# ashawkey/nerf2mesh

Measured on AMD Instinct MI355X. Metric: train_samples_per_sec, higher is better.
Workload: dtype f32 march/composite, f16 autocast encode+MLP (reference -O recipe); 1 GPU; nerf_synthetic/lego stage-0 -O --bound 1 --dt_gamma 0, 800x800 x 100 synthetic views, num_points target 2^18/GPU (adaptive num_rays), occupancy refresh every 16 steps; diffuse_step=1000, refresh_steps_in_window=64, parallelism=single GPU, occupancy_refresh=single GPU, mlp=fused MFMA field kernels, driver=engine.Stage0Engine (fixed launch sequence), pretrain_steps=1000, params=18367240

## Files before the change

### include/n2m_hip.h

```cpp
#ifndef N2M_HIP_H
#define N2M_HIP_H

#include <stdint.h>

#ifdef __cplusplus
extern "C" {
#endif

#define N2M_ABI_VERSION 1

enum { N2M_F32 = 0, N2M_F16 = 1 };

enum {
    N2M_OK = 0,
    N2M_EINVAL = -1,
    N2M_ENULL = -2,
    N2M_EUNSUPPORTED = -3
};

int n2m_abi_version(void);
const char* n2m_last_error(void);


int n2m_near_far_from_aabb(const float* rays_o, const float* rays_d, const float* aabb, uint32_t N,
// ... 104 lines not shown

uint64_t n2m_grid_binned_workspace_bytes(uint32_t B, uint32_t D, uint32_t C, uint32_t max_level,
                                         const int32_t* host_offsets, int dtype, int tv);
int n2m_grid_encode_backward_binned(const void* grad, const float* inputs, const int32_t* host_offsets,
                                    void* grad_embeddings, uint32_t B, uint32_t D, uint32_t C, uint32_t L,
                                    uint32_t max_level, float S, uint32_t H, uint32_t gridtype, int align_corners,
                                    uint32_t interp, int dtype, const float* tv_embeddings, float tv_weight,
                                    float tv_weight_outer, float tv_inner01, const float* tv_scale,
                                    float* found_inf, void* workspace, uint64_t workspace_bytes, void* stream);
int n2m_grad_total_variation_binned(const float* inputs, const float* embeddings, float* grad,
                                    const int32_t* host_offsets, float weight, float weight_outer, float inner01,
                                    const float* weight_scale, uint32_t B, uint32_t D, uint32_t C, uint32_t L, float S,
                                    uint32_t H, uint32_t gridtype, int align_corners, void* workspace,
                                    uint64_t workspace_bytes, void* stream);

int n2m_grid_encode_forward_pair(const float* inputs, const float* embeddings1, const void* embeddings2,
                                 const int32_t* offsets, float* outputs1, void* outputs2, uint32_t B, uint32_t L,
                                 uint32_t max_level, float S, uint32_t H, uint32_t gridtype, int align_corners,
                                 uint32_t interp, float in_scale, float in_offset, void* stream);

int n2m_grid_encode_forward_packed(const float* inputs, const void* packed, const int32_t* offsets, float* outputs1,
                                   void* outputs2, uint32_t B, uint32_t L, uint32_t max_level, float S, uint32_t H,
                                   uint32_t gridtype, int align_corners, uint32_t interp, float in_scale, float in_offset,
                                   void* stream);
int n2m_grid_encode_forward_packed_tv(const float* inputs, const void* packed, const int32_t* offsets, float* outputs1,
                                      void* outputs2, uint32_t B, uint32_t L, uint32_t max_level, float S, uint32_t H,
                                      uint32_t gridtype, int align_corners, uint32_t interp, float in_scale, float in_offset,
                                      float* tv_corners, void* stream);
int n2m_grid_encode_forward_packed_tvterms(const float* inputs, const void* packed, const int32_t* offsets, float* outputs1,
                                           void* outputs2, uint32_t B, uint32_t L, uint32_t max_level, float S, uint32_t H,
                                           uint32_t gridtype, int align_corners, uint32_t interp, float in_scale, float in_offset,
                                           float tv_weight, float tv_weight_outer, float tv_inner01, const float* tv_scale,
                                           float* tv_out, void* stream);
int n2m_grid_backward_tv_corners(const float* tv_corners);

int n2m_grid_encode_forward_packed_levels(const float* inputs, const void* packed, const int32_t* offsets, float* outputs1,
                                          void* outputs2, uint32_t B, uint32_t L, uint32_t max_level, float S, uint32_t H,
                                          uint32_t gridtype, int align_corners, uint32_t interp, float in_scale, float in_offset,
                                          uint32_t level_begin, uint32_t n_levels, void* stream);

uint64_t n2m_grid_binned_pair_workspace_bytes(uint32_t B, uint32_t max_level, const int32_t* host_offsets);
int n2m_grid_encode_backward_binned_pair(const float* grad1, const void* grad2, const float* inputs,
                                         const int32_t* host_offsets, float* grad_embeddings1,
                                         void* grad_embeddings2, uint32_t B, uint32_t L, uint32_t max_level, float S,
                                         uint32_t H, uint32_t gridtype, int align_corners, uint32_t interp,
                                         const float* tv_embeddings, float tv_weight, float tv_weight_outer,
                                         float tv_inner01, const float* tv_scale, float* found_inf, float in_scale,
                                         float in_offset, int overwrite, void* workspace, uint64_t workspace_bytes,
                                         void* stream);
int n2m_grid_encode_backward_binned_pair_half(const float* grad1, const void* grad2, const float* inputs,
                                         const int32_t* host_offsets, float* grad_embeddings1,
                                         void* grad_embeddings2, uint32_t B, uint32_t L, uint32_t max_level, float S,
                                         uint32_t H, uint32_t gridtype, int align_corners, uint32_t interp,
                                         const float* tv_embeddings, float tv_weight, float tv_weight_outer,
                                         float tv_inner01, const float* tv_scale, float* found_inf, float in_scale,
                                         float in_offset, int overwrite, void* workspace, uint64_t workspace_bytes,
                                         void* stream, int half);

typedef struct {
    const float* p_in[2]; const float* m_in[2]; const float* v_in[2];
    float* p_out[2]; float* m_out[2]; float* v_out[2];
    void* packed;
    uint32_t first_level;
    float lr[2]; int32_t slot[2];
    double beta1, beta2; float eps;
    const float* scale; const float* bias;
// ... 238 lines not shown
    float lambda_entropy; int alpha_mode;
    float* depth; const float* gt_depth; const float* depth_weight; float lambda_depth;
    int32_t* live; uint32_t* block_live;
} N2mCompositeLoss;
int n2m_composite_loss_train(const N2mCompositeLoss* d, void* stream);

int n2m_sample_order_live_first(const int32_t* rays, const int32_t* live, const uint32_t* block_live, uint32_t N, uint32_t M,
                                uint32_t* perm, void* stream);
int n2m_grid_backward_sample_order(const uint32_t* perm);

int n2m_grid_backward_merge_levels(uint32_t levels);

#define N2M_ADAM_MAX 16
typedef struct {
    void* param[N2M_ADAM_MAX]; const void* grad[N2M_ADAM_MAX]; void* exp_avg[N2M_ADAM_MAX]; void* exp_avg_sq[N2M_ADAM_MAX];
    void* half_shadow[N2M_ADAM_MAX];
    uint32_t numel[N2M_ADAM_MAX]; float lr[N2M_ADAM_MAX]; int32_t grad_is_half[N2M_ADAM_MAX];
    int32_t shadow_mode[N2M_ADAM_MAX];
    int32_t clear_grad[N2M_ADAM_MAX];
    int32_t slot[N2M_ADAM_MAX];
    uint32_t count;
} N2mAdamDesc;
int n2m_adam_step(const N2mAdamDesc* desc, double beta1, double beta2, float eps, const float* scale,
                  const float* found_inf, const float* bias, void* stream);
#define N2M_EMA_MAX 16
typedef struct {
    void* shadow[N2M_EMA_MAX]; const void* param[N2M_EMA_MAX];
    uint32_t numel[N2M_EMA_MAX];
    uint32_t count;
} N2mEmaDesc;
int n2m_ema_update(const N2mEmaDesc* desc, float one_minus_decay, void* stream);

#define N2M_TAIL_TICKET_WORDS (64 * 32)
typedef struct {
    float* growth_tracker; float* steps;
    uint32_t participants; float growth_factor, backoff_factor, growth_interval;
    const float* loss_partial; uint32_t n_partial; uint32_t n_rays; float* loss; float* loss_sum;
    const float* extra_partial; uint32_t n_extra; float extra_scale;
    const float* extra2_partial; uint32_t n_extra2; float extra2_scale;
    uint32_t* ticket;
} N2mScalerTail;
int n2m_scaler_update_slots(float* scale, float* found_inf, float* bias, double beta1, double beta2, const N2mScalerTail* tail, void* stream);

int n2m_adam_step_scaler(const N2mAdamDesc* desc, double beta1, double beta2, float eps, float* scale, float* found_inf, float* bias,
                         const N2mScalerTail* tail, void* stream);

int n2m_sdf_offsets(const float* xyz, uint32_t M, float eps, float bound, float* pts, float* pts01, void* stream);
int n2m_sdf_alpha_forward(const float* sdf, const float* sdf6, const float* dirs, const float* ts, uint32_t M, const float* variance, float eps,
                          float cos_anneal_ratio, float* alpha, float* normal, float* eik_partial, void* stream);
int n2m_sdf_alpha_backward(const float* d_alpha, const float* sdf, const float* sdf6, const float* dirs, const float* ts, uint32_t M,
                           const float* variance, float eps, float cos_anneal_ratio, const float* seed, float eik_coef, float* d_sdf,
                           float* d_sdf6, float* var_partial, float* d_variance, float* found_inf, void* stream);


int n2m_sh_encode_forward(const float* inputs, float* outputs, uint32_t B, uint32_t D, uint32_t degree,
                          float* dy_dx, void* stream);

int n2m_sh_encode_backward(const float* grad, const float* inputs, uint32_t B, uint32_t D, uint32_t degree,
                           const float* dy_dx, float* grad_inputs, void* stream);


enum {
    N2M_K_GRID_FWD = 0, N2M_K_GRID_BWD, N2M_K_GRID_TV, N2M_K_MARCH_COUNT, N2M_K_MARCH_WRITE,
    N2M_K_COMPOSITE_FWD, N2M_K_COMPOSITE_BWD, N2M_K_NEAR_FAR, N2M_K_PACKBITS, N2M_K_MLP_FWD, N2M_K_MLP_BWD,
    N2M_K_RASTER, N2M_K_GRID_FWD_PACKED , N2M_K_ADAM,
    N2M_K_INTERP_FWD, N2M_K_INTERP_BWD, N2M_K_AA_FWD, N2M_K_AA_BWD, N2M_K_RASTER_BWD, N2M_K_COUNT
};
int n2m_prof_enable(int on);
int n2m_prof_reset(void);
int n2m_prof_read(int kernel_id, uint64_t* launches, double* total_ms, double* algo_bytes);
int n2m_prof_seen(int kernel_id, uint64_t* launches_seen);
const char* n2m_prof_name(int kernel_id);

// ... 7 lines not shown
```

### include/n2m_mlp.h

```cpp
#ifndef N2M_MLP_H
#define N2M_MLP_H

#include <stdint.h>

#ifdef __cplusplus
extern "C" {
#endif

int n2m_field_forward(const float* xyz, const float* dirs, const float* h1, const void* h2, const float* w_sigma0,
                      const float* w_sigma1, const float* w_color0, const float* w_color1, const float* w_color2,
                      const float* w_spec0, const float* w_spec1, uint32_t M, int shading, int normalize_dirs, float* sigma, float* rgb,
                      float* specular, void* stream);

int n2m_field_backward(const float* xyz, const float* dirs, const float* h1, const void* h2, const float* w_sigma0,
                       const float* w_sigma1, const float* w_color0, const float* w_color1, const float* w_color2,
                       const float* w_spec0, const float* w_spec1, uint32_t M, int shading, int normalize_dirs, const float* d_sigma,
                       const float* d_rgb, const float* d_specular, float* d_h1, void* d_h2, float* d_w_sigma0,
                       float* d_w_sigma1, float* d_w_color0, float* d_w_color1, float* d_w_color2, float* d_w_spec0,
                       float* d_w_spec1, float* found_inf, void* stream);

int n2m_field_forward_train(const float* xyz, const float* dirs, const float* h1, const void* h2, const float* w_sigma0,
                            const float* w_sigma1, const float* w_color0, const float* w_color1, const float* w_color2,
                            const float* w_spec0, const float* w_spec1, uint32_t M, int shading, int normalize_dirs, float* sigma, float* rgb,
                            float* specular, float* spec_sq_partial, void* stream);
int n2m_field_backward_train(const float* xyz, const float* dirs, const float* h1, const void* h2, const float* w_sigma0,
                             const float* w_sigma1, const float* w_color0, const float* w_color1, const float* w_color2,
                             const float* w_spec0, const float* w_spec1, uint32_t M, int shading, int normalize_dirs, const float* d_sigma,
                             const float* d_rgb, const float* d_specular, float* d_h1, void* d_h2, float* d_w_sigma0,
                             float* d_w_sigma1, float* d_w_color0, float* d_w_color1, float* d_w_color2, float* d_w_spec0,
                             float* d_w_spec1, float* found_inf, float spec_reg, const float* seed, void* stream);
uint32_t n2m_field_spec_partials(void);

typedef struct N2mDwSum {
    const float* partial;
    uint32_t n_rows, mask;
    float* dw[7];
    float* found_inf;
} N2mDwSum;
int n2m_field_backward_defer_dw(N2mDwSum* out);
int n2m_field_dw_sum(const N2mDwSum* d, void* stream);
int n2m_grid_backward_dw_rider(const N2mDwSum* d, int* carried);

uint32_t n2m_field_ind_max_dim(void);
uint64_t n2m_field_ind_workspace_bytes(uint32_t M, uint32_t R);
int n2m_field_sample_views(const int32_t* rays, const int32_t* ray_view, uint32_t N, uint32_t M, int32_t* sample_view, void* stream);
int n2m_field_forward_ind(const float* xyz, const float* dirs, const float* h1, const void* h2, const float* w_sigma0,
                          const float* w_sigma1, const float* w_color0, const float* w_color1, const float* w_color2,
                          const float* w_spec0, const float* w_spec1, const float* codes, const int32_t* sample_view, uint32_t R, uint32_t D,
                          uint32_t M, int shading, int normalize_dirs, float* sigma, float* rgb, float* specular, void* stream);
int n2m_field_forward_ind_train(const float* xyz, const float* dirs, const float* h1, const void* h2, const float* w_sigma0,
                                const float* w_sigma1, const float* w_color0, const float* w_color1, const float* w_color2,
                                const float* w_spec0, const float* w_spec1, const float* codes, const int32_t* sample_view, uint32_t R,
                                uint32_t D, uint32_t M, int shading, int normalize_dirs, float* sigma, float* rgb, float* specular,
                                float* spec_sq_partial, void* stream);
int n2m_field_backward_ind(const float* xyz, const float* dirs, const float* h1, const void* h2, const float* w_sigma0,
                           const float* w_sigma1, const float* w_color0, const float* w_color1, const float* w_color2,
                           const float* w_spec0, const float* w_spec1, const float* codes, const int32_t* sample_view, uint32_t R, uint32_t D,
                           uint32_t M, int shading, int normalize_dirs, const float* d_sigma, const float* d_rgb, const float* d_specular,
                           float* d_h1, void* d_h2, float* d_w_sigma0, float* d_w_sigma1, float* d_w_color0, float* d_w_color1,
                           float* d_w_color2, float* d_w_spec0, float* d_w_spec1, float* d_codes, void* workspace, uint64_t workspace_bytes,
                           float* found_inf, void* stream);
int n2m_field_backward_ind_train(const float* xyz, const float* dirs, const float* h1, const void* h2, const float* w_sigma0,
                                 const float* w_sigma1, const float* w_color0, const float* w_color1, const float* w_color2,
                                 const float* w_spec0, const float* w_spec1, const float* codes, const int32_t* sample_view, uint32_t R,
// ... 10 lines not shown
```

### nerf2mesh_amd/_lib.py

```python
import ctypes
import os
import threading

_HERE = os.path.dirname(os.path.abspath(__file__))
LIB_PATH = os.environ.get("N2M_HIP_LIB") or os.path.join(_HERE, "lib", "libn2m_hip.so")

_u32, _i32, _f32, _vp, _int, _u64 = ctypes.c_uint32, ctypes.c_int32, ctypes.c_float, ctypes.c_void_p, ctypes.c_int, ctypes.c_uint64

SIGNATURES = {
    "n2m_near_far_from_aabb": [_vp, _vp, _vp, _u32, _f32, _vp, _vp, _vp],
    "n2m_sph_from_ray": [_vp, _vp, _f32, _u32, _vp, _vp],
    "n2m_morton3D": [_vp, _u32, _vp, _vp],
    "n2m_morton3D_invert": [_vp, _u32, _vp, _vp],
    "n2m_packbits": [_vp, _u32, _f32, _vp, _vp],
    "n2m_packbits_dev": [_vp, _u32, _vp, _vp, _vp],
    "n2m_flatten_rays": [_vp, _u32, _u32, _vp, _vp],
    "n2m_march_rays_train": [_vp, _vp, _vp, _f32, _int, _f32, _u32, _u32, _u32, _u32, _vp, _vp, _vp, _vp, _vp, _vp, _vp, _vp, _vp],
    "n2m_march_rays_train_write": [_vp, _vp, _vp, _f32, _int, _f32, _u32, _u32, _u32, _u32, _vp, _vp, _vp, _vp, _vp, _vp, _vp, _u32, _vp],
    "n2m_march_rays_train_fused": [_vp, _vp, _vp, _f32, _int, _f32, _u32, _u32, _u32, _u32, _vp, _vp, _vp, _vp, _vp, _vp, _vp, _vp, _u32, _vp, _u64, _vp],
    "n2m_march_fused_workspace_bytes": [_u32],
    "n2m_march_fallback_count": [_vp],
    "n2m_debug_fill_times": [_int, _vp],
    "n2m_stream_copy": [_vp, _vp, _u64, _u32, _vp],
    "n2m_sample_order_live_first": [_vp, _vp, _vp, _u32, _u32, _vp, _vp],
# ... 89 lines not shown
    "n2m_uv_project": [_vp, _vp, _vp, _vp, _u32, _u32, _vp, _vp, _vp],
    "n2m_uv_sum_f64": [_vp, _u32, _vp, _vp],
    "n2m_uv_rects": [_vp, _u32, ctypes.c_double, _i32, _vp, _vp, _vp],
    "n2m_uv_shelf_pack": [_vp, _vp, _u32, _i32, _i32, _vp, _vp, _vp],
    "n2m_uv_write_vt": [_vp, _vp, _vp, _vp, _u32, ctypes.c_double, _i32, _i32, _i32, _vp, _vp],
    "n2m_uv_canvas_evict": [_vp, _vp, _u32, _i32, _i32, _vp, _vp, _vp],
    "n2m_uv_face_metrics": [_vp, _vp, _vp, _u32, _i32, _i32, _vp, _vp, _vp],
    "n2m_texture_pad_nearest": [_vp, _vp, _u32, _u32, _u32, _u32, _vp],
    "n2m_asset_shade": [_vp, _vp, _vp, _vp, _vp, _vp, _vp, _u32, _u32, _u32, _u32, _int, _int, _vp, _vp],
    "n2m_freq_encode_forward": [_vp, _u32, _u32, _u32, _u32, _vp, _vp],
    "n2m_freq_encode_backward": [_vp, _vp, _u32, _u32, _u32, _u32, _vp, _vp],
    "n2m_get_rays": [_vp, _vp, _vp, _u32, _u32, _u32, _f32, _f32, _f32, _f32, _vp, _vp, _vp, _vp, _vp],
    "n2m_batch_rays": [_vp, _vp],
    "n2m_batch_views": [_vp, _u32, _u32, _vp, _vp],
    "n2m_depth_bank_fill": [_vp, _u32, _u32, _u32, _u32, _f32, _f32, _f32, _f32, _vp, _vp],
    "n2m_capture_view": [_vp, _u32, _u32, _u32, _u32, _u32, _f32, _f32, _f32, _f32, _vp, _vp, _vp, _vp, _vp, _vp, _u32, _vp],
    "n2m_capture_box_downscale": [_vp, _u32, _u32, _u32, _u32, _vp, _vp],
    "n2m_adam_step": [_vp, ctypes.c_double, ctypes.c_double, _f32, _vp, _vp, _vp, _vp],
    "n2m_adam_step_scaler": [_vp, ctypes.c_double, ctypes.c_double, _f32, _vp, _vp, _vp, _vp, _vp],
    "n2m_ema_update": [_vp, _f32, _vp],
    "n2m_scaler_update_slots": [_vp, _vp, _vp, ctypes.c_double, ctypes.c_double, _vp, _vp],
    "n2m_sdf_offsets": [_vp, _u32, _f32, _f32, _vp, _vp, _vp],
    "n2m_sdf_alpha_forward": [_vp, _vp, _vp, _vp, _u32, _vp, _f32, _f32, _vp, _vp, _vp, _vp],
    "n2m_sdf_alpha_backward": [_vp, _vp, _vp, _vp, _vp, _u32, _vp, _f32, _f32, _vp, _f32, _vp, _vp, _vp, _vp, _vp, _vp],
    "n2m_photo_loss_forward": [_vp, _vp, _vp, _vp, _f32, _f32, _f32, _u32, _vp, _vp, _vp, _vp],
    "n2m_photo_loss_backward": [_vp, _vp, _vp, _vp, _f32, _f32, _f32, _u32, _vp, _vp, _vp, _vp],
    "n2m_sh_encode_forward": [_vp, _vp, _u32, _u32, _u32, _vp, _vp],
    "n2m_sh_encode_backward": [_vp, _vp, _u32, _u32, _u32, _vp, _vp, _vp],
    "n2m_field_forward": [_vp] * 11 + [_u32, _int, _int] + [_vp] * 4,
    "n2m_field_backward": [_vp] * 11 + [_u32, _int, _int] + [_vp] * 14,
    "n2m_field_forward_train": [_vp] * 11 + [_u32, _int, _int] + [_vp] * 5,
    "n2m_field_backward_train": [_vp] * 11 + [_u32, _int, _int] + [_vp] * 13 + [_f32, _vp, _vp],
    "n2m_field_spec_partials": [],
    "n2m_field_backward_defer_dw": [_vp],
    "n2m_field_dw_sum": [_vp, _vp],
    "n2m_grid_backward_dw_rider": [_vp, _vp],
    "n2m_field_ind_max_dim": [],
    "n2m_field_ind_workspace_bytes": [_u32, _u32],
    "n2m_field_sample_views": [_vp, _vp, _u32, _u32, _vp, _vp],
    "n2m_field_forward_ind": [_vp] * 13 + [_u32, _u32, _u32, _int, _int] + [_vp] * 4,
    "n2m_field_forward_ind_train": [_vp] * 13 + [_u32, _u32, _u32, _int, _int] + [_vp] * 5,
    "n2m_field_backward_ind": [_vp] * 13 + [_u32, _u32, _u32, _int, _int] + [_vp] * 14 + [_u64, _vp, _vp],
    "n2m_field_backward_ind_train": [_vp] * 13 + [_u32, _u32, _u32, _int, _int] + [_vp] * 14 + [_u64, _vp, _f32, _vp, _vp],
    "n2m_rasterize_forward": [_vp, _vp, _u32, _u32, _u32, _u32, _vp, _vp, _vp],
    "n2m_rasterize_backward": [_vp, _vp, _vp, _vp, _u32, _u32, _u32, _u32, _vp, _vp],
    "n2m_interpolate_forward": [_vp, _vp, _vp, _u32, _u32, _u32, _u32, _u32, _vp, _vp],
    "n2m_interpolate_backward": [_vp, _vp, _vp, _vp, _u32, _u32, _u32, _u32, _u32, _vp, _vp, _vp],
    "n2m_interpolate_backward_strided": [_vp, _vp, _vp, _vp, _u32, _u32, _u32, _u32, _u32, _u32, _vp, _vp, _vp],
    "n2m_antialias_build_topology": [_vp, _u32, _vp, _u32, _vp],
    "n2m_antialias_forward": [_vp, _vp, _vp, _vp, _vp, _u32, _u32, _u32, _u32, _u32, _u32, _vp, _vp],
    "n2m_antialias_backward": [_vp, _vp, _vp, _vp, _vp, _u32, _vp, _u32, _u32, _u32, _u32, _u32, _f32, _vp, _vp, _vp],
    "n2m_antialias_backward_seeded": [_vp, _vp, _vp, _vp, _vp, _u32, _vp, _u32, _u32, _u32, _u32, _u32, _f32, _vp, _vp, _vp],
    "n2m_to_clip": [_vp, _vp, _u32, _vp, _vp],
    "n2m_to_clip_backward": [_vp, _vp, _u32, _vp, _vp],
    "n2m_laplacian_forward": [_vp, _vp, _vp, _u32, _vp, _f32, _f32, _f32, _u32, _vp, _vp, _vp, _vp],
    "n2m_laplacian_backward": [_vp, _vp, _vp, _vp, _u32, _vp, _f32, _vp, _f32, _f32, _u32, _vp, _vp, _vp],
    "n2m_laplacian_backward_acc": [_vp, _vp, _vp, _vp, _u32, _vp, _f32, _vp, _f32, _f32, _u32, _vp, _vp, _vp],
    "n2m_mesh_losses_forward": [_vp, _vp, _u32, _vp, _u32, _f32, _f32, _vp, _vp],
    "n2m_mesh_losses_backward": [_vp, _vp, _vp, _vp, _u32, _vp, _vp, _vp, _u32, _u32, _vp, _f32, _f32, _vp, _vp],
    "n2m_mesh_losses_backward_acc": [_vp, _vp, _vp, _vp, _u32, _vp, _vp, _vp, _u32, _u32, _vp, _f32, _f32, _vp, _vp],
    "n2m_gather_rows": [_vp, _vp, _u32, _u32, _vp, _vp],
    "n2m_gather_rows_strided": [_vp, _vp, _u32, _u32, _u32, _vp, _u32, _vp],
    "n2m_scatter_rows_strided": [_vp, _vp, _u32, _u32, _u32, _vp, _u32, _vp],
    "n2m_scatter_rows": [_vp, _vp, _u32, _u32, _vp, _vp],
    "n2m_stage1_head": [_vp, _vp, _vp, _u32, _u32, _u32, _vp, _vp, _f32, _f32, _f32, _vp, _vp, _vp, _vp, _vp, _vp, _vp, _vp, _vp, _vp, _int, _vp, _vp, _vp],
    "n2m_peer_alloc": [ctypes.c_size_t, _int, ctypes.POINTER(_vp)],
    "n2m_peer_free": [_vp],
    "n2m_peer_export": [_vp, _vp],
    "n2m_peer_import": [_vp, ctypes.POINTER(_vp)],
    "n2m_peer_unmap": [_vp],
    "n2m_peer_signal": [_vp, _u32, _vp],
    "n2m_peer_wait": [_vp, _u32, _u32, _u32, _u32, _vp, _vp],
    "n2m_peer_copy": [_vp, _vp, ctypes.c_size_t, _vp],
    "n2m_peer_reduce_slices": [_vp, _vp, _u32, _u32, _vp, _vp, _vp, _vp],
    "n2m_adam_step_peer": [_vp, ctypes.c_double, ctypes.c_double, _f32, _vp, _vp, _vp, _vp, _vp],
    "n2m_grid_backward_peer_route": [_vp],
    "n2m_prof_enable": [_int],
    "n2m_prof_reset": [],
    "n2m_prof_read": [_int, ctypes.POINTER(ctypes.c_uint64), ctypes.POINTER(ctypes.c_double), ctypes.POINTER(ctypes.c_double)],
    "n2m_prof_seen": [_int, ctypes.POINTER(ctypes.c_uint64)],
}

RESTYPES = {"n2m_occupancy_update_partials": _u32, "n2m_grid_binned_workspace_bytes": _u64, "n2m_grid_binned_pair_workspace_bytes": _u64, "n2m_march_fused_workspace_bytes": _u64,
            "n2m_marching_cubes_workspace_bytes": _u64, "n2m_field_spec_partials": _u32, "n2m_field_ind_max_dim": _u32,
            "n2m_field_ind_workspace_bytes": _u64}

F32, F16 = 0, 1
ADAM_MAX = 16


class AdamDesc(ctypes.Structure):
    _fields_ = [("param", _vp * ADAM_MAX), ("grad", _vp * ADAM_MAX), ("exp_avg", _vp * ADAM_MAX), ("exp_avg_sq", _vp * ADAM_MAX),
                ("half_shadow", _vp * ADAM_MAX), ("numel", _u32 * ADAM_MAX), ("lr", _f32 * ADAM_MAX), ("grad_is_half", _i32 * ADAM_MAX),
                ("shadow_mode", _i32 * ADAM_MAX), ("clear_grad", _i32 * ADAM_MAX), ("slot", _i32 * ADAM_MAX), ("count", _u32)]


class ScalerTail(ctypes.Structure):
    _fields_ = [("growth_tracker", _vp), ("steps", _vp), ("participants", _u32), ("growth_factor", _f32), ("backoff_factor", _f32),
                ("growth_interval", _f32), ("loss_partial", _vp), ("n_partial", _u32), ("n_rays", _u32), ("loss", _vp), ("loss_sum", _vp),
                ("extra_partial", _vp), ("n_extra", _u32), ("extra_scale", _f32), ("extra2_partial", _vp), ("n_extra2", _u32),
                ("extra2_scale", _f32), ("ticket", _vp)]


class DwSum(ctypes.Structure):
    _fields_ = [("partial", _vp), ("n_rows", _u32), ("mask", _u32), ("dw", _vp * 7), ("found_inf", _vp)]


class BatchRays(ctypes.Structure):
    _fields_ = [("poses", _vp), ("uniforms", _vp), ("V", _u32), ("N", _u32), ("H", _u32), ("W", _u32), ("fx", _f32), ("fy", _f32), ("cx", _f32),
                ("cy", _f32), ("intrinsics", _vp), ("images", _vp), ("bank", _vp), ("lut", _vp), ("depth_bank", _vp), ("coords", _vp),
                ("kp_depth", _vp), ("kp_weight", _vp), ("view", _u32), ("first", _u32), ("aabb", _vp), ("min_near", _f32), ("cam_near_far", _vp),
                ("rays_o", _vp), ("rays_d", _vp), ("rgba", _vp), ("nears", _vp), ("fars", _vp), ("noises", _vp), ("bg", _vp), ("gt_depth", _vp),
                ("depth_weight", _vp), ("counter", _vp)]


class CompositeLoss(ctypes.Structure):
    _fields_ = [("sigmas", _vp), ("rgbs", _vp), ("ts", _vp), ("rays", _vp), ("M", _u32), ("N", _u32), ("T_thresh", _f32), ("gt_rgba", _vp),
                ("bg", _vp), ("bg_scalar", _f32), ("lambda_rgb", _f32), ("lambda_mask", _f32), ("grad_loss", _vp), ("weights_sum", _vp),
                ("image", _vp), ("grad_sigmas", _vp), ("grad_rgbs", _vp), ("partial", _vp), ("ticket", _vp), ("loss", _vp), ("loss_sum", _vp),
                ("lambda_entropy", _f32), ("alpha_mode", _int), ("depth", _vp), ("gt_depth", _vp), ("depth_weight", _vp), ("lambda_depth", _f32),
                ("live", _vp), ("block_live", _vp)]


EMA_MAX = 16


class EmaDesc(ctypes.Structure):
    _fields_ = [("shadow", _vp * EMA_MAX), ("param", _vp * EMA_MAX), ("numel", _u32 * EMA_MAX), ("count", _u32)]


ASSET_MAX = 8


class AssetTable(ctypes.Structure):
# ... 142 lines not shown
```

### nerf2mesh_amd/csrc/gridencoder.hip

```cpp
#include <math.h>
#include <stdlib.h>

#include <atomic>
#include <type_traits>

#include "n2m_common.hpp"
#include "../../include/n2m_peer.h"
#include "../../include/n2m_mlp.h"
#include "n2m_dw_sum.hpp"

namespace {

constexpr uint32_t kMaxLevels = 32;

struct LevelTable {
    float scale[kMaxLevels];
    uint32_t resolution[kMaxLevels];
};

__host__ LevelTable make_levels(uint32_t L, float S, uint32_t H) {
    LevelTable t;
    for (uint32_t l = 0; l < kMaxLevels; ++l) {
        const float sc = l < L ? exp2f((float)l * S) * (float)H - 1.0f : 0.0f;
        t.scale[l] = sc;
        t.resolution[l] = (uint32_t)ceilf(sc) + 1u;
    }
    return t;
}

template <uint32_t D> struct Primes;
__device__ constexpr uint32_t kPrimes[7] = {1u, 2654435761u, 805459861u, 3674653429u, 2097192037u, 1434869437u, 2165219737u};

template <uint32_t D>
struct Indexer {
    uint32_t stride[D];
    uint32_t size;
    uint32_t mask;
    bool hashed, pow2, wrap;

    __device__ __forceinline__ Indexer(uint32_t size_, uint32_t resolution, uint32_t gridtype, bool align_corners) : size(size_) {
        uint32_t s = 1;
#pragma unroll
// ... 326 lines not shown
#pragma unroll
        for (uint32_t d = 0; d < D; ++d) w *= (corner & (1u << d)) ? frac[d] : 1 - frac[d];
#pragma unroll
        for (uint32_t c = 0; c < C; ++c) accum(acc.v[c], w, g[corner].v[c]);
    }
    acc.store(out);
}

template <typename T>
__global__ void zero_levels_kernel(T* __restrict__ outputs, uint32_t B, uint32_t LC, uint32_t first, uint32_t count) {
    const uint64_t t = (uint64_t)blockIdx.x * blockDim.x + threadIdx.x;
    if (t >= (uint64_t)B * count) return;
    const uint32_t b = (uint32_t)(t / count), k = (uint32_t)(t - (uint64_t)b * count);
    outputs[(size_t)b * LC + first + k] = (T)0;
}

__device__ __forceinline__ void atomic_add_row(float* dst, const float* v, uint32_t C) {
    for (uint32_t c = 0; c < C; ++c) unsafeAtomicAdd(dst + c, v[c]);
}

struct TvParams {
    const float* table;
    float weight, weight_outer, inner01;
    const float* scale_ptr;
    uint32_t stride = 1;
    const float* corners = nullptr;
};

__device__ __forceinline__ void tv_weights(const TvParams& tv, float& w_in, float& w_out) {
    float wi = tv.weight, wo = tv.weight_outer;
    if (tv.table && tv.scale_ptr) { const float s = *tv.scale_ptr; wi *= s; wo *= s; }
    w_in = wi / 6.0f; w_out = wo / 6.0f;
}
__device__ __forceinline__ bool tv_inner(const TvParams& tv, const float (&x)[3]) {
    return fmaxf(fmaxf(fabsf(x[0] - 0.5f), fabsf(x[1] - 0.5f)), fabsf(x[2] - 0.5f)) <= tv.inner01;
}
__device__ __forceinline__ float tv_reduce6(float centre, const float (&nb)[6], const bool (&nb_ok)[6], float w) {
    float sum = 0.f, sq = 0.f;
#pragma unroll
    for (uint32_t k = 0; k < 6; ++k)
        if (nb_ok[k]) { const float dv = centre - nb[k]; sum += dv; sq += dv * dv; }
    return w * sum * __builtin_amdgcn_rsqf(sq + 1e-9f);
}

__device__ __forceinline__ float tv_term(const float* __restrict__ tab, const Indexer<3>& ix, uint32_t (&cell)[3], uint32_t here, uint32_t resolution,
                                         float w, uint32_t stride);
template <bool TVT>
__global__ void __launch_bounds__(256)
grid_forward3_packed_kernel(const float* __restrict__ inputs, const uint2* __restrict__ packed, const int32_t* __restrict__ offsets,
                            float* __restrict__ out1, _Float16* __restrict__ out2, uint32_t B, uint32_t max_level, LevelTable lv,
                            uint32_t gridtype, bool align_corners, uint32_t interp, uint32_t n_tiles, float in_scale, float in_offset,
                            uint32_t xcd_group, uint32_t level_begin, uint32_t n_levels, float4* __restrict__ tv4, TvParams tv,
                            float* __restrict__ tv_out) {
    __builtin_amdgcn_s_setprio(3);
    constexpr uint32_t D = 3;
    typedef _Float16 h2 __attribute__((ext_vector_type(2)));
    uint32_t level, tile;
    if (xcd_group == 0u) {
        level = blockIdx.x / n_tiles;
        tile = blockIdx.x - level * n_tiles;
        level += level_begin;
    } else {
        const uint32_t g = xcd_group, groups = 8u / g, per_group = n_levels / groups;
        const uint32_t xcd = blockIdx.x & 7u, k = xcd / g, j = xcd - k * g, i = blockIdx.x >> 3;
        const uint32_t tiles_per_xcd = (n_tiles + g - 1u) / g;
        const uint32_t li = i / tiles_per_xcd;
        tile = (i - li * tiles_per_xcd) * g + j;
        if (li >= per_group || tile >= n_tiles) return;
        const uint32_t pair = k + groups * (li >> 1);
        level = level_begin + ((li & 1u) ? n_levels - 1u - pair : pair);
    }
    if (level >= max_level) return;
    const uint32_t b = tile * 256 + threadIdx.x;
    if (b >= B) return;
    const uint32_t row0 = (uint32_t)offsets[level];
    const uint32_t size = (uint32_t)offsets[level + 1] - row0;
    const float scale = lv.scale[level];
    const Indexer<D> ix(size, lv.resolution[level], gridtype, align_corners);
    const uint2* __restrict__ tab = packed + (size_t)row0;
    float* o1 = out1 + (size_t)level * B + b;
    _Float16* o2 = out2 ? out2 + ((size_t)level * B + b) * 2 : nullptr;

    float x[D];
    load_point<D>(inputs, b, x);
#pragma unroll
    for (uint32_t d = 0; d < D; ++d) x[d] = x[d] * in_scale + in_offset;
// ... 40 lines not shown
            rx1[q] = ((cell[0] + 1u) ^ h) & ix.mask;
            pr[q] = *reinterpret_cast<const uint4*>(tab + (rx[q] & ~1u));
        }
        uint2 extra[4];
        if (!x_even) {
#pragma unroll
            for (uint32_t q = 0; q < 4; ++q) extra[q] = tab[rx1[q]];
        }
        if constexpr (TVT) {
            const uint32_t h00 = hy0 ^ hz0;
            if (x_even) tvm[0] = tabf[(size_t)(cell[0] > 0u ? ((cell[0] - 1u) ^ h00) & ix.mask : rx[0]) * 2u];
            tvm[1] = tabf[(size_t)(cell[1] > 0u ? (cell[0] ^ (hy0 - kPrimes[1]) ^ hz0) & ix.mask : rx[0]) * 2u];
            tvm[2] = tabf[(size_t)(cell[2] > 0u ? (cell[0] ^ hy0 ^ (hz0 - kPrimes[2])) & ix.mask : rx[0]) * 2u];
        }
#pragma unroll
        for (uint32_t q = 0; q < 4; ++q) {
            const bool odd_row = (rx[q] & 1u) != 0u;
            const uint2 lo = make_uint2(pr[q].x, pr[q].y), hi = make_uint2(pr[q].z, pr[q].w);
            g[2 * q] = odd_row ? hi : lo;
            g[2 * q + 1] = x_even ? (odd_row ? lo : hi) : extra[q];
            if constexpr (TVT) { if (q == 0u && !x_even) tvm[0] = __uint_as_float(odd_row ? lo.x : hi.x); }
        }
        if (tv4) tv4[(size_t)level * B + b] = make_float4(__uint_as_float(g[0].x), __uint_as_float(g[1].x), __uint_as_float(g[2].x), __uint_as_float(g[4].x));
    } else {
#pragma unroll
        for (uint32_t corner = 0; corner < 8; ++corner) {
            const uint32_t v[D] = {cell[0] + (corner & 1u), cell[1] + ((corner >> 1) & 1u), cell[2] + (corner >> 2)};
            g[corner] = tab[ix.row(v)];
        }
        tv_fast = false;
    }
    if constexpr (TVT) {
        float w_in, w_out;
        tv_weights(tv, w_in, w_out);
        const float w = tv_inner(tv, x) ? w_in : w_out;
        float tvv;
        if (tv_fast) {
            const float nb[6] = {__uint_as_float(g[1].x), tvm[0], __uint_as_float(g[2].x), tvm[1], __uint_as_float(g[4].x), tvm[2]};
            const bool nb_ok[6] = {cell[0] < tv_res, cell[0] > 0u, cell[1] < tv_res, cell[1] > 0u, cell[2] < tv_res, cell[2] > 0u};
            tvv = tv_reduce6(__uint_as_float(g[0].x), nb, nb_ok, w);
        } else {
            tvv = tv_term(tabf, ix, cell, ix.row(cell), tv_res, w, 2u);
        }
        tv_out[(size_t)level * B + b] = tvv;
    }
    float a1 = 0.0f;
    _Float16 a2[2] = {(_Float16)0, (_Float16)0};
#pragma unroll
    for (uint32_t corner = 0; corner < 8; ++corner) {
        float w = 1.0f;
#pragma unroll
        for (uint32_t d = 0; d < D; ++d) w *= (corner & (1u << d)) ? frac[d] : 1 - frac[d];
        const h2 c2 = __builtin_bit_cast(h2, g[corner].y);
        accum(a1, w, __uint_as_float(g[corner].x));
        accum(a2[0], w, c2.x);
        accum(a2[1], w, c2.y);
    }
    *o1 = a1;
    if (!o2) return;
    Row<_Float16, 2> r2;
    r2.v[0] = a2[0]; r2.v[1] = a2[1];
    r2.store(o2);
}

__global__ void __launch_bounds__(256)
grid_forward3_pair_kernel(const float* __restrict__ inputs, const float* __restrict__ table1, const _Float16* __restrict__ table2,
                          const int32_t* __restrict__ offsets, float* __restrict__ out1, _Float16* __restrict__ out2, uint32_t B,
// ... 3663 lines not shown
    hipStream_t s = (hipStream_t)stream;
    const BinLayout lay = make_bin_plan(B, 2, L, host_offsets, false, kPairP, 2);
    N2M_REQUIRE(lay.ok, N2M_EUNSUPPORTED, "%s: table layout not supported", fn);
    const LevelTable lv = make_levels(L, S, H);
    const TvParams tv{tv_embeddings, tv_weight, tv_weight_outer, tv_inner01, tv_scale, g_cfg_tv_stride.load()};
    N2M_PROF(N2M_K_GRID_TV, s, (double)B * (12.0 + (double)L * 7 * 4.0 + (double)L * 4.0));
    tv_terms_kernel<<<dim3(n2m_ceil_div(B, 256), L), 256, 0, s>>>(inputs, tv, B, B, lay.plan, lv, gridtype, align_corners != 0, interp, in_scale, in_offset, tv_out);
    N2M_CHECK_LAUNCH();
    return 0;
}

extern "C" int n2m_grid_encode_forward_pair(const float* inputs, const float* embeddings1, const void* embeddings2, const int32_t* offsets,
                                            float* outputs1, void* outputs2, uint32_t B, uint32_t L, uint32_t max_level, float S, uint32_t H,
                                            uint32_t gridtype, int align_corners, uint32_t interp, float in_scale, float in_offset,
                                            void* stream) {
    const char* fn = "grid_encode_forward_pair";
    if (int rc = check_dims(fn, 3, 2, L, max_level, N2M_F16)) return rc;
    N2M_REQUIRE(inputs && embeddings1 && embeddings2 && offsets && outputs1 && outputs2, N2M_ENULL, "%s: NULL tensor", fn);
    if (B == 0 || max_level == 0) return 0;
    hipStream_t s = (hipStream_t)stream;
    const LevelTable lv = make_levels(L, S, H);
    N2M_PROF(N2M_K_GRID_FWD, s, (double)B * (12.0 + (double)max_level * 8 * (4 + 4) + (double)max_level * (4 + 4)));
    const uint32_t n_tiles = n2m_ceil_div(B, 256);
    grid_forward3_pair_kernel<<<n_tiles * max_level, 256, 0, s>>>(inputs, embeddings1, (const _Float16*)embeddings2, offsets, outputs1,
                                                                 (_Float16*)outputs2, B, max_level, lv, gridtype, align_corners != 0, interp, n_tiles,
                                                                 in_scale, in_offset);
    N2M_CHECK_LAUNCH();
    return 0;
}

static int forward_packed(const float* inputs, const void* packed, const int32_t* offsets, float* outputs1, void* outputs2, uint32_t B, uint32_t L,
                          uint32_t max_level, float S, uint32_t H, uint32_t gridtype, int align_corners, uint32_t interp, float in_scale, float in_offset,
                          void* stream, uint32_t level_begin, uint32_t n_levels, float* tv_corners = nullptr, const TvParams* tvp = nullptr,
                          float* tv_out = nullptr);

extern "C" int n2m_grid_encode_forward_packed(const float* inputs, const void* packed, const int32_t* offsets, float* outputs1, void* outputs2,
                                              uint32_t B, uint32_t L, uint32_t max_level, float S, uint32_t H, uint32_t gridtype,
                                              int align_corners, uint32_t interp, float in_scale, float in_offset, void* stream) {
    return forward_packed(inputs, packed, offsets, outputs1, outputs2, B, L, max_level, S, H, gridtype, align_corners, interp, in_scale, in_offset, stream, 0u,
                          max_level);
}

extern "C" int n2m_grid_encode_forward_packed_levels(const float* inputs, const void* packed, const int32_t* offsets, float* outputs1, void* outputs2,
                                                     uint32_t B, uint32_t L, uint32_t max_level, float S, uint32_t H, uint32_t gridtype,
                                                     int align_corners, uint32_t interp, float in_scale, float in_offset, uint32_t level_begin,
                                                     uint32_t n_levels, void* stream) {
    N2M_REQUIRE(n_levels >= 1 && level_begin + n_levels <= max_level, N2M_EINVAL,
                "grid_encode_forward_packed_levels: levels [%u, %u) outside [0, %u)", level_begin, level_begin + n_levels, max_level);
    return forward_packed(inputs, packed, offsets, outputs1, outputs2, B, L, max_level, S, H, gridtype, align_corners, interp, in_scale, in_offset, stream,
                          level_begin, n_levels);
}

static int forward_packed(const float* inputs, const void* packed, const int32_t* offsets, float* outputs1, void* outputs2, uint32_t B, uint32_t L,
                          uint32_t max_level, float S, uint32_t H, uint32_t gridtype, int align_corners, uint32_t interp, float in_scale, float in_offset,
                          void* stream, uint32_t level_begin, uint32_t n_levels, float* tv_corners, const TvParams* tvp, float* tv_out) {
    const char* fn = "grid_encode_forward_packed";
    if (int rc = check_dims(fn, 3, 2, L, max_level, N2M_F16)) return rc;
    N2M_REQUIRE(inputs && packed && offsets && outputs1, N2M_ENULL, "%s: NULL tensor", fn);
    N2M_REQUIRE(((uintptr_t)packed & 15u) == 0, N2M_EINVAL, "%s: the packed table must be 16-byte aligned", fn);
    if (B == 0 || max_level == 0) return 0;
    hipStream_t s = (hipStream_t)stream;
    const LevelTable lv = make_levels(L, S, H);
    N2M_PROF_K(outputs2 ? N2M_K_GRID_FWD_PACKED : N2M_K_GRID_FWD, s,
             (outputs2 ? (double)B * (12.0 + (double)n_levels * 8 * (4 + 4) + (double)n_levels * (4 + 4))
                       : (double)B * (12.0 + (double)n_levels * 8 * 4 + (double)n_levels * 4)) + (tv_out ? (double)B * n_levels * (3 * 4.0 + 4.0) : 0.0));
    const uint32_t n_tiles = n2m_ceil_div(B, 256);
    static const uint32_t xg_env = getenv("N2M_FWD_XCD_GROUP") ? (uint32_t)atoi(getenv("N2M_FWD_XCD_GROUP")) : 4u;
    const uint32_t xg = ((n_levels == 16u || n_levels == 8u) && (xg_env == 1u || xg_env == 2u || xg_env == 4u) && n_levels % (2u * (8u / xg_env)) == 0u) ? xg_env : 0u;
    const uint32_t blocks = xg ? 8u * (n_levels / (8u / xg)) * n2m_ceil_div(n_tiles, xg) : n_tiles * n_levels;
    if (tv_out) {
        TvParams tv = *tvp;
        tv.table = reinterpret_cast<const float*>(packed);
        tv.stride = 2u;
        N2M_LAUNCH(grid_forward3_packed_kernel<true>, blocks, 256, 0, s, inputs, (const uint2*)packed, offsets, outputs1, (_Float16*)outputs2, B,
                   level_begin + n_levels, lv, gridtype, align_corners != 0, interp, n_tiles, in_scale, in_offset, xg, level_begin, n_levels,
                   (float4*)nullptr, tv, tv_out);
    } else {
        N2M_LAUNCH(grid_forward3_packed_kernel<false>, blocks, 256, 0, s, inputs, (const uint2*)packed, offsets, outputs1, (_Float16*)outputs2, B,
                   level_begin + n_levels, lv, gridtype, align_corners != 0, interp, n_tiles, in_scale, in_offset, xg, level_begin, n_levels,
                   reinterpret_cast<float4*>(tv_corners), TvParams{}, (float*)nullptr);
    }
    N2M_CHECK_LAUNCH();
    return 0;
}

extern "C" int n2m_grid_encode_forward_packed_tv(const float* inputs, const void* packed, const int32_t* offsets, float* outputs1, void* outputs2,
                                                 uint32_t B, uint32_t L, uint32_t max_level, float S, uint32_t H, uint32_t gridtype, int align_corners,
                                                 uint32_t interp, float in_scale, float in_offset, float* tv_corners, void* stream) {
    N2M_REQUIRE(tv_corners == nullptr || ((uintptr_t)tv_corners & 15u) == 0, N2M_EINVAL, "grid_encode_forward_packed_tv: tv_corners must be 16-byte aligned");
    return forward_packed(inputs, packed, offsets, outputs1, outputs2, B, L, max_level, S, H, gridtype, align_corners, interp, in_scale, in_offset, stream,
                          0u, max_level < L ? max_level : L, tv_corners);
}

extern "C" int n2m_grid_encode_forward_packed_tvterms(const float* inputs, const void* packed, const int32_t* offsets, float* outputs1, void* outputs2,
                                                      uint32_t B, uint32_t L, uint32_t max_level, float S, uint32_t H, uint32_t gridtype,
                                                      int align_corners, uint32_t interp, float in_scale, float in_offset, float tv_weight,
                                                      float tv_weight_outer, float tv_inner01, const float* tv_scale, float* tv_out, void* stream) {
    N2M_REQUIRE(tv_out != nullptr, N2M_ENULL, "grid_encode_forward_packed_tvterms: NULL tv_out");
    N2M_REQUIRE(max_level == L, N2M_EINVAL, "grid_encode_forward_packed_tvterms: TV terms need max_level == L (every level of tv_out is written)");
    const TvParams tv{nullptr, tv_weight, tv_weight_outer, tv_inner01, tv_scale, 2u};
    return forward_packed(inputs, packed, offsets, outputs1, outputs2, B, L, max_level, S, H, gridtype, align_corners, interp, in_scale, in_offset, stream,
                          0u, L, nullptr, &tv, tv_out);
}

extern "C" int n2m_debug_fill_times(int on, unsigned long long* out) {
    if (out) N2M_HIP(hipMemcpyFromSymbol(out, HIP_SYMBOL(g_fill_t), sizeof(unsigned long long) * 96));
    if (out) N2M_HIP(hipMemcpyFromSymbol(out + 96, HIP_SYMBOL(g_acc_t), sizeof(unsigned long long) * 20));
    const unsigned int v = (unsigned int)on;
    N2M_HIP(hipMemcpyToSymbol(HIP_SYMBOL(g_fill_timing_on), &v, sizeof(v)));
    g_fill_dbg_host = v;
    return 0;
}

extern "C" int n2m_grid_backward_peer_route(const N2mPeerRoute* route) {
    if (!route) { g_peer_route = N2mPeerRoute{}; return 0; }
    N2M_REQUIRE(route->world >= 1 && route->world <= N2M_PEER_MAX && route->rows_c > 0 && route->rows_f > 0 &&
                (uint64_t)route->world * route->rows_c >= route->split_row && (uint64_t)(route->world - 1u) * route->rows_c < route->split_row,
                N2M_EINVAL, "grid_backward_peer_route: 1..%d ranks, (world - 1) * rows_c < split_row <= world * rows_c", N2M_PEER_MAX);
    for (int h = 0; h < 2; ++h)
        for (uint32_t r = 0; r < route->world; ++r)
            N2M_REQUIRE(route->g1[h][r] && route->g2[h][r], N2M_ENULL, "grid_backward_peer_route: NULL staging slot (half %d, owner %u)", h, r);
    g_peer_route = *route;
    return 0;
}

extern "C" int n2m_grid_backward_config(int tv_stride, float overflow_div) {
    N2M_REQUIRE((tv_stride == 1 || tv_stride == 2) && overflow_div >= 1.0f, N2M_EINVAL, "grid_backward_config: tv_stride 1 or 2, overflow_div >= 1");
    g_cfg_tv_stride.v = (uint32_t)tv_stride;
    g_cfg_overflow_div.v = overflow_div;
    return 0;
}
```

### nerf2mesh_amd/csrc/mlp.hip

```cpp
#include <map>
#include <mutex>

#include "n2m_common.hpp"
#include "../../include/n2m_mlp.h"
#include "n2m_dw_sum.hpp"

namespace {

typedef _Float16 h4 __attribute__((ext_vector_type(4)));
typedef float f16x __attribute__((ext_vector_type(16)));

#define MFMA(a, b, c) __builtin_amdgcn_mfma_f32_32x32x8f16((a), (b), (c), 0, 0, 0)
typedef _Float16 h8 __attribute__((ext_vector_type(8)));
#define MFMA16(a, b, c) __builtin_amdgcn_mfma_f32_32x32x16_f16((a), (b), (c), 0, 0, 0)

constexpr int P_S0 = 28, P_S1 = 36, P_C0 = 44, P_C1 = 68, P_C2 = 68, P_P0 = 12, P_P1 = 36;
constexpr int P_S1T = 12, P_S0T = 36, P_C2T = 12, P_C1T = 68, P_C0T = 68, P_P1T = 12, P_P0T = 36;
constexpr int O_S0 = 0;
constexpr int O_S1 = O_S0 + 32 * P_S0;
constexpr int O_C0 = O_S1 + 32 * P_S1;
constexpr int O_C1 = O_C0 + 64 * P_C0;
constexpr int O_C2 = O_C1 + 64 * P_C1;
constexpr int O_P0 = O_C2 + 32 * P_C2;
constexpr int O_P1 = O_P0 + 32 * P_P0;
constexpr int FWD_HALVES = O_P1 + 32 * P_P1;
constexpr int O_S1T = FWD_HALVES;
constexpr int O_S0T = O_S1T + 32 * P_S1T;
constexpr int O_C2T = O_S0T + 32 * P_S0T;
constexpr int O_C1T = O_C2T + 64 * P_C2T;
constexpr int O_C0T = O_C1T + 64 * P_C1T;
constexpr int O_P1T = O_C0T + 64 * P_C0T;
constexpr int O_P0T = O_P1T + 32 * P_P1T;
constexpr int ALL_W_HALVES = O_P0T + 32 * P_P0T;
constexpr int TILE_PITCH = 68;
constexpr int TILE_HALVES = 32 * TILE_PITCH;
constexpr int BWD_HALVES = ALL_W_HALVES + 4 * 2 * TILE_HALVES;
constexpr int BWD_PC_TILES_HALVES = ALL_W_HALVES + 4 * 4 * TILE_HALVES;
constexpr int BWD_PC_HALVES = BWD_PC_TILES_HALVES > 65536 ? BWD_PC_TILES_HALVES : 65536;
// ... 312 lines not shown
    for (int i = 0; i < 8; ++i) { asm volatile("" : "+v"(r.h1v[i])); asm volatile("" : "+v"(r.h2v[i])); }
#pragma unroll
    for (int i = 0; i < 3; ++i) { asm volatile("" : "+v"(r.xyz[i])); asm volatile("" : "+v"(r.dir[i])); asm volatile("" : "+v"(r.drgb[i])); asm volatile("" : "+v"(r.dspec[i])); }
    asm volatile("" : "+v"(r.dsig));
}
__device__ __forceinline__ void density_frags(const RawTile& r, h4 (&b)[3]) {
#pragma unroll
    for (int kb = 0; kb < 2; ++kb)
#pragma unroll
        for (int i = 0; i < 4; ++i) b[kb][i] = (_Float16)r.h1v[4 * kb + i];
    b[2] = zero4();
    b[2][0] = (_Float16)r.xyz[0]; b[2][1] = (_Float16)r.xyz[1]; b[2][2] = (_Float16)r.xyz[2];
}
__device__ __forceinline__ void color_frags(const RawTile& r, h4 (&b)[5]) {
#pragma unroll
    for (int kb = 0; kb < 4; ++kb) {
        const u2v_t v = {r.h2v[2 * kb], r.h2v[2 * kb + 1]};
        b[kb] = __builtin_bit_cast(h4, v);
    }
    b[4] = zero4();
    b[4][0] = (_Float16)r.xyz[0]; b[4][1] = (_Float16)r.xyz[1]; b[4][2] = (_Float16)r.xyz[2];
}
template <typename P>
__device__ __forceinline__ void dir_frag(const FieldArgs& a, const RawTile& r, P& bp) {
    float d0 = r.dir[0], d1 = r.dir[1], d2 = r.dir[2];
    if (a.normalize_dirs) {
        const float nn = sqrtf(fmaxf((d0 * d0 + d1 * d1) + d2 * d2, 1e-20f));
        d0 /= nn; d1 /= nn; d2 /= nn;
    }
    bp[0] = (_Float16)d0; bp[1] = (_Float16)d1; bp[2] = (_Float16)d2;
}

template <bool DO_DENSITY, bool DO_COLOR, bool IND = false>
__global__ void __launch_bounds__(256) field_forward_kernel(typename ArgsOf<IND>::type a) {
    __builtin_amdgcn_s_setprio(3);
    extern __shared__ __attribute__((aligned(16))) _Float16 lds[];
    stage_images<256, false, DO_DENSITY, DO_COLOR, IND>(lds, a);
    if constexpr (IND) stage_color0_ind<false>(lds + O_C0X_FWD, nullptr, a.w[2], a.ind.D);

    const int lane = threadIdx.x & 63, n = lane & 31, g = lane >> 5;
    const uint32_t wave = blockIdx.x * 4 + (threadIdx.x >> 6), n_waves = gridDim.x * 4;
    const uint32_t n_tiles = (a.M + 31) / 32;
    RawTile nxt;
    float spec_sq = 0.f;
    fetch_tile<DO_DENSITY, DO_COLOR, false>(a, wave, n, g, nxt);
    for (uint32_t tile = wave; tile < n_tiles; tile += n_waves) {
        const uint32_t s = tile * 32 + n;
        const bool valid = s < a.M;
        settle_tile(nxt);
        const RawTile cur = nxt;
        fetch_tile<DO_DENSITY, DO_COLOR, false>(a, tile + n_waves, n, g, nxt);
        if (DO_DENSITY) {
            h4 b0[3];
            density_frags(cur, b0);
            f16x d = zero16();
            d = mm_k<3>(lds + O_S0, P_S0, 0, b0, d, lane);
            const h4 b1[4] = {relu_pack<0>(d), relu_pack<1>(d), relu_pack<2>(d), relu_pack<3>(d)};
            f16x o = zero16();
            o = mm_k<4>(lds + O_S1, P_S1, 0, b1, o, lane);
            if (valid && g == 0) a.sigma[s] = a.raw_density ? (float)(_Float16)o[0] : expf((float)(_Float16)o[0]);
        }
        if (DO_COLOR) {
            h4 b0[5];
            color_frags(cur, b0);
            f16x d1[2] = {zero16(), zero16()};
            h4 bc[2];
            if constexpr (IND) code_frags(a.ind, s, valid, g, bc);
#pragma unroll
            for (int mb = 0; mb < 2; ++mb) {
                if constexpr (IND) {
                    d1[mb] = mm_k<5>(lds + O_C0X_FWD, P_C0X, mb, b0, d1[mb], lane);
                    d1[mb] = MFMA16(cat8(ld_a(lds + O_C0X_FWD, P_C0X, mb, 5, lane), ld_a(lds + O_C0X_FWD, P_C0X, mb, 6, lane)), cat8(bc[0], bc[1]), d1[mb]);
                } else
                d1[mb] = mm_k<5>(lds + O_C0, P_C0, mb, b0, d1[mb], lane);
// ... 14 lines not shown
                h4 bp = zero4();
                if (g == 0) {
                    if (valid) dir_frag(a, cur, bp);
                    bp[3] = (_Float16)q3;
                } else { bp[0] = (_Float16)q0; bp[1] = (_Float16)q1; }
                f16x p1 = MFMA(ld_a(lds + O_P0, P_P0, 0, 0, lane), bp, zero16());
                const h4 bq[4] = {relu_pack<0>(p1), relu_pack<1>(p1), relu_pack<2>(p1), relu_pack<3>(p1)};
                f16x p2 = zero16();
                p2 = mm_k<4>(lds + O_P1, P_P1, 0, bq, p2, lane);
                const float s0 = sigmoid_h(p2[0]), s1 = sigmoid_h(p2[1]), s2 = sigmoid_h(p2[2]);
                if (valid && g == 0 && a.specular) {
                    a.specular[(size_t)s * 3] = s0; a.specular[(size_t)s * 3 + 1] = s1; a.specular[(size_t)s * 3 + 2] = s2;
                }
                if (valid && g == 0) spec_sq += (s0 * s0 + s1 * s1) + s2 * s2;
                if (a.shading == 2) { cr = s0; cg = s1; cb = s2; }
                else {
                    cr = fminf(fmaxf((float)(_Float16)(s0 + q0), 0.f), 1.f);
                    cg = fminf(fmaxf((float)(_Float16)(s1 + q1), 0.f), 1.f);
                    cb = fminf(fmaxf((float)(_Float16)(s2 + q2), 0.f), 1.f);
                }
            }
            if (valid && g == 0 && a.rgb) {
                a.rgb[(size_t)s * 3] = cr; a.rgb[(size_t)s * 3 + 1] = cg; a.rgb[(size_t)s * 3 + 2] = cb;
            }
        }
    }
    if (DO_COLOR && a.spec_sq_partial) {
        __shared__ float spec_wave[4];
        const float w = n2m_wave_sum(spec_sq);
        if (lane == 0) spec_wave[threadIdx.x >> 6] = w;
        __syncthreads();
        if (threadIdx.x == 0) a.spec_sq_partial[blockIdx.x] = ((spec_wave[0] + spec_wave[1]) + spec_wave[2]) + spec_wave[3];
        if (blockIdx.x == 0)
            for (int i = (int)gridDim.x + (int)threadIdx.x; i < kSpecPartials; i += 256) a.spec_sq_partial[i] = 0.f;
    }
}

__device__ __forceinline__ void tile_put(_Float16* tile, int kb, const h4& f, int lane) {
    *reinterpret_cast<h4*>(tile + (lane & 31) * TILE_PITCH + 8 * kb + 4 * (lane >> 5)) = f;
}
__device__ __forceinline__ h4 tile_get(const _Float16* tile, int kq, int fb, int lane) {
    const _Float16* p = tile + (8 * kq + 4 * (lane >> 5)) * TILE_PITCH + 32 * fb + (lane & 31);
    h4 r;
    r[0] = p[0]; r[1] = p[TILE_PITCH]; r[2] = p[2 * TILE_PITCH]; r[3] = p[3 * TILE_PITCH];
    return r;
}
typedef short s4v_t __attribute__((__vector_size__(8)));
__device__ __forceinline__ h4 tile_get_tr(const _Float16* tile, int kq, int fb, int lane) {
    const _Float16* p = tile + (8 * kq + 4 * (lane >> 5) + ((lane & 15) >> 2)) * TILE_PITCH + 32 * fb + 16 * ((lane >> 4) & 1) + 4 * (lane & 3);
    return __builtin_bit_cast(h4, __builtin_amdgcn_ds_read_tr16_b64_v4i16((__attribute__((address_space(3))) s4v_t*)p));
}
template <int MB, int NB, bool TR = false>
__device__ __forceinline__ void dw_tile(f16x (&acc)[MB][NB], const _Float16* tY, const _Float16* tX, int lane) {
    if constexpr (TR) {
        h4 ay[4][MB], bx[4][NB];
#pragma unroll
        for (int kq = 0; kq < 4; ++kq) {
#pragma unroll
            for (int mb = 0; mb < MB; ++mb) ay[kq][mb] = tile_get_tr(tY, kq, mb, lane);
#pragma unroll
            for (int nb = 0; nb < NB; ++nb) bx[kq][nb] = tile_get_tr(tX, kq, nb, lane);
        }
#pragma unroll
        for (int kq = 0; kq < 4; kq += 2)
#pragma unroll
            for (int mb = 0; mb < MB; ++mb)
#pragma unroll
                for (int nb = 0; nb < NB; ++nb)
// ... 633 lines not shown
}

int check_field(const char* fn, const float* xyz, const float* h1, const float* const* w, bool density, int shading) {
    N2M_REQUIRE(shading >= 0 && shading <= 2, N2M_EINVAL, "%s: shading must be 0 (diffuse), 1 (full) or 2 (specular)", fn);
    N2M_REQUIRE(xyz, N2M_ENULL, "%s: xyz is NULL", fn);
    if (density) N2M_REQUIRE(h1 && w[0] && w[1], N2M_ENULL, "%s: density branch needs h1 and sigma_net weights", fn);
    return 0;
}

float* dw_scratch(hipStream_t s, bool ind = false) {
    static std::mutex mu;
    static std::map<std::pair<int, hipStream_t>, float*> plain, wide;
    auto& bufs = ind ? wide : plain;
    std::lock_guard<std::mutex> lk(mu);
    int dev = 0;
    if (hipGetDevice(&dev) != hipSuccess) return nullptr;
    const auto key = std::make_pair(dev, s);
    auto it = bufs.find(key);
    if (it != bufs.end()) return it->second;
    float* p = nullptr;
    if (hipMalloc((void**)&p, (size_t)256 * (ind ? kDwTotalInd : kDwTotal) * sizeof(float)) != hipSuccess) return nullptr;
    bufs[key] = p;
    return p;
}

uint32_t persistent_grid(uint32_t M) {
    const uint32_t tiles = (M + 31) / 32;
    const uint32_t need = (tiles + 3) / 4;
    return need < 256u ? (need ? need : 1u) : 256u;
}

}

static int field_forward_impl(const float* xyz, const float* dirs, const float* h1, const void* h2, const float* w_sigma0,
                                 const float* w_sigma1, const float* w_color0, const float* w_color1, const float* w_color2,
                                 const float* w_spec0, const float* w_spec1, uint32_t M, int shading, int normalize_dirs, float* sigma, float* rgb,
                                 float* specular, float* spec_sq_partial, void* stream, const IndArgs* ind = nullptr) {
    const float* w[7] = {w_sigma0, w_sigma1, w_color0, w_color1, w_color2, w_spec0, w_spec1};
    const bool density = sigma != nullptr;
    if (int rc = check_field("field_forward", xyz, h1, w, density, shading)) return rc;
    const bool color = rgb != nullptr;
    N2M_REQUIRE(density || color, N2M_ENULL, "field_forward: both sigma and rgb are NULL");
    if (color) {
        N2M_REQUIRE(h2 && w[2] && w[3] && w[4], N2M_ENULL, "field_forward: colour branch needs h2 and color_net weights");
        if (shading != 0) N2M_REQUIRE(dirs && w[5] && w[6], N2M_ENULL, "field_forward: shading != 0 needs dirs and specular_net weights");
    }
    if (M == 0) return 0;
    FieldArgs a{};
    a.xyz = xyz; a.dirs = dirs; a.h1 = h1; a.h2 = (const _Float16*)h2; a.normalize_dirs = normalize_dirs & 1; a.raw_density = (normalize_dirs >> 1) & 1;
    for (int i = 0; i < 7; ++i) a.w[i] = w[i];
    a.M = M; a.shading = shading; a.sigma = sigma; a.rgb = rgb; a.specular = specular;
    a.spec_sq_partial = (color && shading != 0) ? spec_sq_partial : nullptr;
    hipStream_t s = (hipStream_t)stream;
    N2M_PROF_K(N2M_K_MLP_FWD, s, (double)M * (12 + 64 + 4 + (color ? 64 + 12 + 12 + 12 : 0)));
    const size_t smem = (size_t)FWD_HALVES * 2;
    if (ind && color) {
        FieldArgsInd ai{};
        static_cast<FieldArgs&>(ai) = a;
        ai.ind = *ind;
        const size_t smem_ind = (size_t)(FWD_HALVES + C0X_HALVES) * 2;
        if (density) N2M_LAUNCH((field_forward_kernel<true, true, true>), persistent_grid(M) * 2, 256, smem_ind, s, ai);
        else N2M_LAUNCH((field_forward_kernel<false, true, true>), persistent_grid(M) * 2, 256, smem_ind, s, ai);
        N2M_CHECK_LAUNCH();
        return 0;
    }
    if (color && density) N2M_LAUNCH((field_forward_kernel<true, true>), persistent_grid(M) * 2, 256, smem, s, a);
    else if (color) N2M_LAUNCH((field_forward_kernel<false, true>), persistent_grid(M) * 2, 256, smem, s, a);
    else N2M_LAUNCH((field_forward_kernel<true, false>), persistent_grid(M) * 2, 256, smem, s, a);
    N2M_CHECK_LAUNCH();
    return 0;
}

extern "C" int n2m_field_forward(const float* xyz, const float* dirs, const float* h1, const void* h2, const float* w_sigma0,
                                 const float* w_sigma1, const float* w_color0, const float* w_color1, const float* w_color2,
                                 const float* w_spec0, const float* w_spec1, uint32_t M, int shading, int normalize_dirs, float* sigma, float* rgb,
                                 float* specular, void* stream) {
    return field_forward_impl(xyz, dirs, h1, h2, w_sigma0, w_sigma1, w_color0, w_color1, w_color2, w_spec0, w_spec1, M, shading, normalize_dirs,
                              sigma, rgb, specular, nullptr, stream);
}
extern "C" int n2m_field_forward_train(const float* xyz, const float* dirs, const float* h1, const void* h2, const float* w_sigma0,
                                       const float* w_sigma1, const float* w_color0, const float* w_color1, const float* w_color2,
                                       const float* w_spec0, const float* w_spec1, uint32_t M, int shading, int normalize_dirs, float* sigma,
                                       float* rgb, float* specular, float* spec_sq_partial, void* stream) {
    return field_forward_impl(xyz, dirs, h1, h2, w_sigma0, w_sigma1, w_color0, w_color1, w_color2, w_spec0, w_spec1, M, shading, normalize_dirs,
                              sigma, rgb, specular, spec_sq_partial, stream);
}
extern "C" uint32_t n2m_field_spec_partials(void) { return (uint32_t)kSpecPartials; }

static thread_local N2mDwSum* g_defer_dw = nullptr;
extern "C" int n2m_field_backward_defer_dw(N2mDwSum* out) {
    g_defer_dw = out;
    if (out) *out = N2mDwSum{};
    return 0;
}
static int check_dw_sum(const char* fn, const N2mDwSum* d) {
    N2M_REQUIRE(d != nullptr && d->partial != nullptr, N2M_ENULL, "%s: NULL description / partial rows", fn);
    N2M_REQUIRE(d->n_rows >= 1, N2M_EINVAL, "%s: no partial rows", fn);
    N2M_REQUIRE((d->mask & ~0x7Fu) == 0, N2M_EINVAL, "%s: mask names seven tensors", fn);
    for (int i = 0; i < 7; ++i)
        N2M_REQUIRE(!((d->mask >> i) & 1u) || d->dw[i] != nullptr, N2M_ENULL, "%s: tensor %d is in the mask and NULL", fn, i);
    return 0;
}
extern "C" int n2m_field_dw_sum(const N2mDwSum* d, void* stream) {
    if (int rc = check_dw_sum("field_dw_sum", d)) return rc;
    DwOut o;
    for (int i = 0; i < 7; ++i) o.dw[i] = d->dw[i];
    N2M_LAUNCH(dw_finalize_kernel, kDwSumBlocks, 1024, 0, (hipStream_t)stream, d->partial, d->n_rows, o, d->mask, d->found_inf);
    N2M_CHECK_LAUNCH();
    return 0;
}

static int field_backward_impl(const float* xyz, const float* dirs, const float* h1, const void* h2, const float* w_sigma0,
                                  const float* w_sigma1, const float* w_color0, const float* w_color1, const float* w_color2,
                                  const float* w_spec0, const float* w_spec1, uint32_t M, int shading, int normalize_dirs, const float* d_sigma,
                                  const float* d_rgb, const float* d_specular, float* d_h1, void* d_h2, float* d_w_sigma0,
                                  float* d_w_sigma1, float* d_w_color0, float* d_w_color1, float* d_w_color2, float* d_w_spec0,
                                  float* d_w_spec1, float* found_inf, float spec_reg, const float* seed, void* stream,
                                  const IndArgs* ind = nullptr, float* d_codes = nullptr, long long* code_acc = nullptr) {
// ... 181 lines not shown
```

### nerf2mesh_amd/csrc/step_helpers.hip

```cpp
#include <string.h>

#include "n2m_common.hpp"
#include "../../include/n2m_peer.h"

namespace {

struct RayTerm {
    float e[3];
    float m;
    float bg[3];
};

__device__ __forceinline__ RayTerm ray_term(const float* __restrict__ image, const float* __restrict__ wsum,
                                            const float* __restrict__ gt, const float* __restrict__ bg, float bg_scalar, uint32_t r) {
    RayTerm t;
    const float4 g = *reinterpret_cast<const float4*>(gt + (size_t)r * 4);
    const float a = g.w, ws = wsum[r];
    const float gc[3] = {g.x, g.y, g.z};
#pragma unroll
    for (int c = 0; c < 3; ++c) {
        t.bg[c] = bg ? bg[(size_t)r * 3 + c] : bg_scalar;
        const float target = gc[c] * a + t.bg[c] * (1.0f - a);
        const float pred = image[(size_t)r * 3 + c] + (1.0f - ws) * t.bg[c];
        t.e[c] = pred - target;
    }
    t.m = ws - a;
    return t;
}

__global__ void __launch_bounds__(256)
photo_loss_forward_kernel(const float* __restrict__ image, const float* __restrict__ wsum, const float* __restrict__ gt,
                          const float* __restrict__ bg, float bg_scalar, float lambda_rgb, float lambda_mask, uint32_t N,
                          float* __restrict__ partial, uint32_t* __restrict__ ticket, float* __restrict__ loss) {
    __shared__ float wave_sum[4];
    __shared__ bool last;
    const uint32_t r = blockIdx.x * 256 + threadIdx.x, lane = threadIdx.x & 63u, wid = threadIdx.x >> 6;
// ... 801 lines not shown
                               const float* gt_rgba, const float* bg, float bg_scalar, float lambda_rgb, float lambda_mask, float* image,
                               float* depth, float* weights_sum, float* trig_id, float* loss_px, float* d_alpha, float* d_rgb, float* partial,
                               float* tri_err, float* tri_cnt, int packed_rgba, const float* seed, float* d_copy, void* stream) {
    N2M_REQUIRE(aa_alpha && aa_rgb && rast && gt_rgba && image && depth && weights_sum && trig_id && loss_px && partial, N2M_ENULL,
                "stage1_head: NULL tensor");
    N2M_REQUIRE((d_alpha == nullptr) == (d_rgb == nullptr), N2M_ENULL, "stage1_head: d_alpha and d_rgb come together");
    N2M_REQUIRE((tri_err == nullptr) == (tri_cnt == nullptr), N2M_ENULL, "stage1_head: tri_err and tri_cnt come together");
    N2M_REQUIRE(ssaa == 1 || ssaa == 2, N2M_EUNSUPPORTED, "stage1_head: ssaa 1 or 2 (the reduction is the exact 2 x 2 mean of torch's bilinear minification)");
    N2M_REQUIRE(h0 > 0 && w0 > 0 && (uint64_t)h0 * w0 < (1ull << 31), N2M_EINVAL, "stage1_head: bad image size");
    N2M_REQUIRE(!packed_rgba || !d_rgb || (d_alpha == d_rgb + 3 && ((uintptr_t)d_rgb & 15u) == 0), N2M_EINVAL,
                "stage1_head: packed gradients are ONE 16-byte aligned [h, w, 4] image (d_alpha = d_rgb + 3)");
    N2M_REQUIRE(!d_copy || (packed_rgba && d_rgb && ((uintptr_t)d_copy & 15u) == 0), N2M_EINVAL, "stage1_head: d_copy goes with the packed gradient image");
    hipStream_t s = (hipStream_t)stream;
    const uint32_t N = h0 * w0;
    if (ssaa == 1)
        stage1_head_kernel<1><<<n2m_ceil_div(N, 256), 256, 0, s>>>(aa_alpha, aa_rgb, rast, h0, w0, gt_rgba, bg, bg_scalar, lambda_rgb, lambda_mask,
                                                                  image, depth, weights_sum, trig_id, loss_px, d_alpha, d_rgb, partial, tri_err, tri_cnt, packed_rgba ? 4u : 1u,
                                                                  packed_rgba ? 4u : 3u, seed, d_copy);
    else
        stage1_head_kernel<2><<<n2m_ceil_div(N, 256), 256, 0, s>>>(aa_alpha, aa_rgb, rast, h0, w0, gt_rgba, bg, bg_scalar, lambda_rgb, lambda_mask,
                                                                  image, depth, weights_sum, trig_id, loss_px, d_alpha, d_rgb, partial, tri_err, tri_cnt, packed_rgba ? 4u : 1u,
                                                                  packed_rgba ? 4u : 3u, seed, d_copy);
    N2M_CHECK_LAUNCH();
    return 0;
}

template <bool PEER>
__global__ void __launch_bounds__(256)
adam_kernel(AdamTensors t, float beta1, float beta2, float omb1, float omb2, float eps, const float* scale, const float* found_inf,
            const float* bias, AdamPeerK pe) {
    adam_body<PEER>(t, beta1, beta2, omb1, omb2, eps, scale, found_inf, bias, pe);
}

struct ScalerTailK {
    float* scale; float* growth_tracker; float* found_inf; float* steps; float* bias;
    uint32_t participants; double beta1, beta2; float growth_factor, backoff_factor, growth_interval;
    const float* loss_partial; uint32_t n_partial; float inv_rays; float* loss; float* loss_sum;
    const float* extra_partial; uint32_t n_extra; float extra_scale;
    const float* extra2_partial; uint32_t n_extra2; float extra2_scale;
    uint32_t* ticket;
};

template <bool ONE_WAVE>
__device__ __forceinline__ void scaler_update_slots_body(const ScalerTailK& k) {
    const uint32_t s = ONE_WAVE ? (threadIdx.x & 63u) : threadIdx.x;
    float tot_part = 0.0f, tot_extra = 0.0f, tot_extra2 = 0.0f;
    bool ok;
    if constexpr (ONE_WAVE) {
        auto sum256 = [&](const float* __restrict__ part, uint32_t n) {
            float acc[4] = {0.0f, 0.0f, 0.0f, 0.0f};
            for (uint32_t base = 0; base < n; base += 2048u) {
                float x[8][4];
#pragma unroll
                for (uint32_t k = 0; k < 8u; ++k)
#pragma unroll
                    for (uint32_t w = 0; w < 4u; ++w) {
                        const uint32_t i = base + 256u * k + 64u * w + s;
                        x[k][w] = i < n ? part[i] : 0.0f;
                    }
#pragma unroll
                for (uint32_t k = 0; k < 8u; ++k)
#pragma unroll
                    for (uint32_t w = 0; w < 4u; ++w)
                        if (base + 256u * k + 64u * w + s < n) acc[w] += x[k][w];
            }
            float tot = 0.0f;
#pragma unroll
            for (uint32_t w = 0; w < 4u; ++w) tot += n2m_wave_sum(acc[w]);
            return tot;
        };
        if (k.extra2_partial) tot_extra2 = sum256(k.extra2_partial, k.n_extra2);
        if (k.extra_partial) tot_extra = sum256(k.extra_partial, k.n_extra);
        if (k.loss_partial) tot_part = sum256(k.loss_partial, k.n_partial);
        ok = *k.found_inf == 0.0f;
    } else {
        __shared__ float wave_part[16], wave_extra[16], wave_extra2[16];
        if (k.extra2_partial) {
            float acc = 0.0f;
            for (uint32_t i = s; i < k.n_extra2; i += blockDim.x) acc += k.extra2_partial[i];
            acc = n2m_wave_sum(acc);
            if ((s & 63u) == 0u) wave_extra2[s >> 6] = acc;
        }
        if (k.extra_partial) {
            float acc = 0.0f;
            for (uint32_t i = s; i < k.n_extra; i += blockDim.x) acc += k.extra_partial[i];
            acc = n2m_wave_sum(acc);
            if ((s & 63u) == 0u) wave_extra[s >> 6] = acc;
        }
        if (k.loss_partial) {
            float acc = 0.0f;
            for (uint32_t i = s; i < k.n_partial; i += blockDim.x) acc += k.loss_partial[i];
            acc = n2m_wave_sum(acc);
            if ((s & 63u) == 0u) wave_part[s >> 6] = acc;
        }
        ok = *k.found_inf == 0.0f;
        __syncthreads();
        if (s == 0) {
            for (uint32_t w = 0; w < (blockDim.x + 63u) / 64u; ++w) {
                if (k.loss_partial) tot_part += wave_part[w];
                if (k.extra_partial) tot_extra += wave_extra[w];
                if (k.extra2_partial) tot_extra2 += wave_extra2[w];
            }
        }
    }
    if (k.loss_partial && s == 0) {
        float v = tot_part * k.inv_rays;
        if (k.extra_partial) v += tot_extra * k.extra_scale;
        if (k.extra2_partial) v += tot_extra2 * k.extra2_scale;
        if (k.loss) *k.loss = v;
        if (k.loss_sum) *k.loss_sum += v;
    }
    if (s == 0) {
        if (!ok) {
            if (k.scale) *k.scale *= k.backoff_factor;
            if (k.growth_tracker) *k.growth_tracker = 0.0f;
        } else if (k.growth_tracker) {
            const float g = *k.growth_tracker + 1.0f;
            if (g >= k.growth_interval) {
                const float ns = *k.scale * k.growth_factor;
                if (k.scale && ns <= 3.0e38f) *k.scale = ns;
                *k.growth_tracker = 0.0f;
            } else {
                *k.growth_tracker = g;
            }
        }
        *k.found_inf = 0.0f;
    }
    if (s <= N2M_ADAM_MAX) {
        if (ok && (s == 0 || ((k.participants >> (s - 1u)) & 1u))) k.steps[s] += 1.0f;
        const double t = (double)k.steps[s] + 1.0;
        k.bias[2u * s] = (float)(1.0 - pow(k.beta1, t));
        k.bias[2u * s + 1u] = (float)sqrt(1.0 - pow(k.beta2, t));
    }
}


constexpr uint32_t kTailSlots = 64;
struct AdamTailArgs {
    AdamTensors t; float beta1, beta2, omb1, omb2, eps; const float* scale; const float* found_inf; const float* bias; ScalerTailK tail;
};

__global__ void __launch_bounds__(256) __attribute__((amdgpu_num_sgpr(48)))
adam_kernel_with_scaler(AdamTensors t, float beta1, float beta2, float omb1, float omb2, float eps, const float* scale, const float* found_inf,
                        const float* bias, ScalerTailK tail) {
    adam_body<false>(t, beta1, beta2, omb1, omb2, eps, scale, found_inf, bias, AdamPeerK{});
    if (blockIdx.x != gridDim.x - 1u || threadIdx.x >= 64u) {
        if ((threadIdx.x & 63u) == 0u)
            (void)__hip_atomic_fetch_add(tail.ticket + 32u * (blockIdx.x & (kTailSlots - 1u)), 1u, __ATOMIC_RELAXED, __HIP_MEMORY_SCOPE_AGENT);
        return;
    }
    uint32_t off = (uint32_t)offsetof(AdamTailArgs, tail);
    asm volatile("" : "+s"(off));
    const ScalerTailK* tp = reinterpret_cast<const ScalerTailK*>((const char*)__builtin_amdgcn_kernarg_segment_ptr() + off);
    {
        const uint32_t expected = 4u * gridDim.x - 1u;
        uint32_t* mine = tp->ticket + 32u * threadIdx.x;
        for (;;) {
            uint32_t v = 0u;
#pragma unroll
            for (uint32_t k = 0; k < kTailSlots / 64u; ++k) v += __hip_atomic_load(mine + 32u * 64u * k, __ATOMIC_RELAXED, __HIP_MEMORY_SCOPE_AGENT);
            if (n2m_wave_sum_u32(v) >= expected) break;
            __builtin_amdgcn_s_sleep(8);
        }
#pragma unroll
        for (uint32_t k = 0; k < kTailSlots / 64u; ++k) __hip_atomic_store(mine + 32u * 64u * k, 0u, __ATOMIC_RELAXED, __HIP_MEMORY_SCOPE_AGENT);
    }
    const ScalerTailK k = *tp;
    scaler_update_slots_body<true>(k);
}

static ScalerTailK scaler_tail_k(float* scale, float* found_inf, float* bias, double beta1, double beta2, const N2mScalerTail* t) {
    const bool lp = t->loss_partial != nullptr;
    const float* e1 = lp ? t->extra_partial : nullptr;
    const float* e2 = lp ? t->extra2_partial : nullptr;
    return ScalerTailK{scale, t->growth_tracker, found_inf, t->steps, bias, t->participants, beta1, beta2, t->growth_factor, t->backoff_factor,
                       t->growth_interval, t->loss_partial, lp ? t->n_partial : 0u, lp ? 1.0f / (float)t->n_rays : 0.0f, lp ? t->loss : nullptr,
                       lp ? t->loss_sum : nullptr, e1, e1 ? t->n_extra : 0u, t->extra_scale, e2, e2 ? t->n_extra2 : 0u, t->extra2_scale, t->ticket};
}

static int adam_step_impl(const N2mAdamDesc* d, double beta1, double beta2, float eps, const float* scale, const float* found_inf,
                          const float* bias, const N2mAdamPeer* peer, void* stream, const N2mScalerTail* tail = nullptr) {
    N2M_REQUIRE(d != nullptr && bias != nullptr, N2M_ENULL, "adam_step: NULL descriptor / bias");
    N2M_REQUIRE(d->count >= 1 && d->count <= N2M_ADAM_MAX, N2M_EINVAL, "adam_step: 1..%d tensors per call (got %u)", N2M_ADAM_MAX, d->count);
    AdamTensors t;
    memset(&t, 0, sizeof(t));
    uint32_t blocks = 0;
    for (uint32_t k = 0; k < d->count; ++k) {
        N2M_REQUIRE(d->param[k] && d->grad[k] && d->exp_avg[k] && d->exp_avg_sq[k], N2M_ENULL, "adam_step: NULL tensor %u", k);
        N2M_REQUIRE((((uintptr_t)d->param[k] | (uintptr_t)d->grad[k] | (uintptr_t)d->exp_avg[k] | (uintptr_t)d->exp_avg_sq[k]) & 3u) == 0,
                    N2M_EINVAL, "adam_step: tensor %u is not 4-byte aligned (param/grad/exp_avg/exp_avg_sq)", k);
        t.p[k] = (uint64_t)d->param[k]; t.g[k] = (uint64_t)d->grad[k]; t.m[k] = (uint64_t)d->exp_avg[k]; t.v[k] = (uint64_t)d->exp_avg_sq[k];
        t.shadow[k] = (uint64_t)d->half_shadow[k];
        t.n[k] = d->numel[k];
        t.lr[k] = d->lr[k];
        t.first_block[k] = blocks;
        blocks += n2m_ceil_div(d->numel[k], 1024);
        if (d->grad_is_half[k]) t.g_half_mask |= 1u << k;
        if (d->clear_grad[k] && !d->grad_is_half[k]) t.clear_mask |= 1u << k;
        t.shadow_mode[k] = (uint8_t)(d->half_shadow[k] ? (d->shadow_mode[k] ? d->shadow_mode[k] : 1) : 0);
        N2M_REQUIRE(d->slot[k] >= 0 && d->slot[k] <= N2M_ADAM_MAX, N2M_EINVAL, "adam_step: slot of tensor %u out of range", k);
        t.slot[k] = (uint8_t)d->slot[k];
        N2M_REQUIRE(t.shadow_mode[k] <= 3 && !(t.shadow_mode[k] == 3 && (d->numel[k] & 1u)), N2M_EINVAL, "adam_step: bad shadow mode for tensor %u", k);
    }
    for (uint32_t k = 0; k < d->count; ++k) t.partner[k] = -1;
    for (uint32_t k = 0; k < d->count; ++k) {
        if (t.shadow_mode[k] != 3) continue;
        for (uint32_t j = 0; j < d->count; ++j)
            if (t.shadow_mode[j] == 2 && d->half_shadow[j] == d->half_shadow[k] && d->numel[k] == 2 * d->numel[j] && ((uintptr_t)d->half_shadow[k] & 15u) == 0) {
                N2M_REQUIRE(!((t.clear_mask >> j) & 1u), N2M_EUNSUPPORTED,
                            "adam_step: tensor %u shares a packed table with tensor %u and cannot use clear_grad", j, k);
                t.partner[k] = (int8_t)j;
// ... 62 lines not shown
                                                                        found_inf, bias, pe);
        else
            N2M_LAUNCH((adam_kernel<false>), blocks, 256, 0, (hipStream_t)stream, t, (float)beta1, (float)beta2, (float)(1.0 - beta1), (float)(1.0 - beta2), eps, scale,
                                                                         found_inf, bias, pe);
    }
    N2M_CHECK_LAUNCH();
    return 0;
}

extern "C" int n2m_adam_step(const N2mAdamDesc* d, double beta1, double beta2, float eps, const float* scale, const float* found_inf,
                             const float* bias, void* stream) {
    return adam_step_impl(d, beta1, beta2, eps, scale, found_inf, bias, nullptr, stream);
}

extern "C" int n2m_adam_step_scaler(const N2mAdamDesc* d, double beta1, double beta2, float eps, float* scale, float* found_inf, float* bias,
                                    const N2mScalerTail* tail, void* stream) {
    N2M_REQUIRE(tail != nullptr, N2M_ENULL, "adam_step_scaler: NULL tail (use n2m_adam_step + n2m_scaler_update_slots)");
    return adam_step_impl(d, beta1, beta2, eps, scale, found_inf, bias, nullptr, stream, tail);
}

extern "C" int n2m_adam_step_peer(const N2mAdamDesc* d, double beta1, double beta2, float eps, const float* scale, const float* found_inf,
                                  const float* bias, const N2mAdamPeer* peer, void* stream) {
    N2M_REQUIRE(peer != nullptr, N2M_ENULL, "adam_step_peer: NULL peer description (use n2m_adam_step)");
    return adam_step_impl(d, beta1, beta2, eps, scale, found_inf, bias, peer, stream);
}

__global__ void scaler_update_slots_kernel(const ScalerTailK k) {
    __builtin_amdgcn_s_setprio(3);
    scaler_update_slots_body<false>(k);
}

extern "C" int n2m_scaler_update_slots(float* scale, float* found_inf, float* bias, double beta1, double beta2, const N2mScalerTail* tail,
                                       void* stream) {
    N2M_REQUIRE(tail != nullptr, N2M_ENULL, "scaler_update_slots: NULL tail");
    N2M_REQUIRE(found_inf != nullptr && tail->steps != nullptr && bias != nullptr, N2M_ENULL, "scaler_update_slots: NULL found_inf / steps / bias");
    N2M_REQUIRE(tail->loss_partial == nullptr || tail->n_rays > 0, N2M_EINVAL, "scaler_update_slots: the loss partials need the ray count");
    scaler_update_slots_kernel<<<1, tail->loss_partial ? 256 : 64, 0, (hipStream_t)stream>>>(scaler_tail_k(scale, found_inf, bias, beta1, beta2, tail));
    N2M_CHECK_LAUNCH();
    return 0;
}

struct EmaTensors {
    uint64_t shadow[N2M_EMA_MAX], param[N2M_EMA_MAX];
    uint32_t n[N2M_EMA_MAX], first_block[N2M_EMA_MAX + 1];
    uint32_t count;
};

__global__ void __launch_bounds__(256) ema_update_kernel(EmaTensors t, float one_minus_decay) {
    uint32_t k = 0;
    while (k + 1 < t.count && blockIdx.x >= t.first_block[k + 1]) ++k;
    const uint32_t i0 = ((blockIdx.x - t.first_block[k]) * 256u + threadIdx.x) * 4u;
    const uint32_t n = t.n[k];
    if (i0 >= n) return;
    float* __restrict__ S = reinterpret_cast<float*>(t.shadow[k]);
    const float* __restrict__ P = reinterpret_cast<const float*>(t.param[k]);
    typedef float f4v __attribute__((ext_vector_type(4)));
    if (i0 + 4u <= n && (((t.shadow[k] | t.param[k]) & 15u) == 0)) {
        f4v s = __builtin_nontemporal_load(reinterpret_cast<const f4v*>(S + i0));
        const f4v p = __builtin_nontemporal_load(reinterpret_cast<const f4v*>(P + i0));
        s.x = s.x - (s.x - p.x) * one_minus_decay; s.y = s.y - (s.y - p.y) * one_minus_decay;
        s.z = s.z - (s.z - p.z) * one_minus_decay; s.w = s.w - (s.w - p.w) * one_minus_decay;
        __builtin_nontemporal_store(s, reinterpret_cast<f4v*>(S + i0));
    } else {
        for (uint32_t e = 0; e < 4u && i0 + e < n; ++e) S[i0 + e] = S[i0 + e] - (S[i0 + e] - P[i0 + e]) * one_minus_decay;
    }
}

extern "C" int n2m_ema_update(const N2mEmaDesc* d, float one_minus_decay, void* stream) {
    N2M_REQUIRE(d != nullptr, N2M_ENULL, "ema_update: NULL descriptor");
// ... 22 lines not shown
```

### nerf2mesh_amd/engine.py

```python
import ctypes
import os
import time

import numpy as np
import torch

from . import _lib as L
from . import raymarching, synthetic
from .fused import SHADING, _affine
from .gridencoder import _host_offsets, same_geometry
from .optim import FusedAdamAMP

_p = L.ptr


def _shard_refresh_default():
    from .parallel import shard_refresh_default
    return shard_refresh_default()


def lr_lambda(it, iters):
    return 0.01 + 0.99 * (it / 500) if it <= 500 else 0.1 ** ((it - 500) / (iters - 500))


def peer_chunk_rows(split, world, pad=0):
    if split % 4 != 0 or pad % 4 != 0:
        return None
    cs = (split + 4 * world - 1) // (4 * world) * 4 + pad
    return cs if (world - 1) * cs < split else None


class _RayBufs:

    def __init__(self, cap, dev):
        self.cap = cap
        f = lambda *s: torch.empty(*s, dtype=torch.float32, device=dev)
        self.o, self.d, self.rgba = f(cap, 3), f(cap, 3), f(cap, 4)
        self.nears, self.fars, self.noises, self.bg_buf = f(cap), f(cap), f(cap), f(cap, 3)
        self.gtd, self.dw = f(cap), f(cap)
        self.depth_view = None
        self.u = self.bg = None
        self.rays = torch.empty(cap, 2, dtype=torch.int32, device=dev)
        self.views = None
        self.counter = torch.zeros(1, dtype=torch.int32, device=dev)
        self.ws = torch.empty(int(L.lib().n2m_march_fused_workspace_bytes(cap)), dtype=torch.uint8, device=dev)
        self.one_pass = False
        self.host_count = torch.empty(1, dtype=torch.int32, pin_memory=True)
        self.count_ready = torch.cuda.Event()
        self.written = torch.cuda.Event()
        self.spec = False
        self.index = 0
        self.M = None
        self.loss = torch.empty(1, dtype=torch.float32, device=dev)
        self.samples = None
        self.cap_m = 0
        self.N = 0
        self.args = None
        self.refreshed = False


class Stage0Engine:
    def __init__(self, model, opt, poses, device, rank=0, world_size=1, seed=0, ema_decay=0.95, capture=None):
        self.model, self.opt, self.device = model.to(device), opt, torch.device(device)
        dev = self.device
        self.capture = capture
        if capture is not None:
            capture.check_device(dev)
            poses = capture.poses
        assert dev.type == "cuda", "the step executor drives HIP kernels: no CPU path"
        if bool(opt.sdf) and world_size > 1:
            raise ValueError("Stage0Engine runs the SDF recipe on one rank; use trainer.Stage0Trainer for multi-rank SDF training")
        self.ind_dim = int(getattr(opt, "ind_dim", 0))
        if self.ind_dim > 0 and capture is not None and len(capture) > int(opt.ind_num):
            raise ValueError(f"the capture has {len(capture)} views but ind_num is {int(opt.ind_num)}: every view needs a code row")
        if not self.supported(model, opt, capture=capture, world_size=world_size):
            raise ValueError("Stage0Engine covers the fused recipes (fused_mlp, fp16, individual codes only on a capture -- density mode, "
                             "one rank, ind_dim <= 16 --, power-of-two bound, shared encoder geometry); use trainer.Stage0Trainer for "
                             "other configurations")
        L.lib()
        self.poses = poses.to(dev).float().contiguous()
        self.rank, self.world = rank, world_size
        self.global_step = 0
        self.num_rays = opt.num_rays
        self.gen = torch.Generator(device=dev)
        self.gen.manual_seed(seed + rank)
        self.optimizer = FusedAdamAMP(model.get_params(opt.lr), eps=1e-15, amp=True)
        self.ema = None
        self.epoch_len = max(1, int(poses.shape[0]))
        if ema_decay is not None:
            from .ema import ExponentialMovingAverage
            self.ema = ExponentialMovingAverage(model.parameters(), decay=ema_decay)
# ... 94 lines not shown
                f32 = lambda *sh: torch.empty(*sh, dtype=torch.float32, device=dev)
                f16 = lambda *sh: torch.empty(*sh, dtype=torch.float16, device=dev)
                self.g1s = {"c": f32(self._Cs, 1), "f": f32(self._Fs, 1)}
                self.g2s = {"c": f16(self._Cs, 2), "f": f16(self._Fs, 2)}
                self._inplace_gather = dist.get_backend() == "nccl"
                self.chunked_gather = os.environ.get("N2M_CHUNKED_GATHER", "1") != "0"
        self._bwd_cfg = (2 if self.shard else 1, float(world_size))
        self.peer = None
        if self.shard and os.environ.get("N2M_PEER_STORE", "0") == "1":
            if opt.sdf:
                raise ValueError("N2M_PEER_STORE covers the NeRF recipes (the SDF head's folded backward is not routed)")
            from .parallel import PeerExchange
            self.peer = PeerExchange(rank, world_size, self.rows, self._split, self._Cs, self._Fs, dev, small_n=self.dw.numel() + 1)
            self._peer_small = torch.empty(self.dw.numel() + 1, dtype=torch.float32, device=dev)
            pk = model.packed_tables()
            self.peer.packed.copy_(pk)
            model._packed = self.peer.packed
            model._packed_buffer = self.peer.packed
            self._peer_route = self.peer.route()
            self._peer_fused = (os.environ.get("N2M_PEER_FUSED", "1") != "0" and self._Cs % 4 == 0 and self._Fs % 4 == 0 and self._split % 2 == 0)
            self._adam_peer = None
        if self.shard:
            self.optimizer.shard_sync = lambda: self.sync_parameters(moments=True)
        self.sdf_fold = os.environ.get("N2M_SDF_FOLD", "1") != "0"
        self.sdf_tv_all = os.environ.get("N2M_SDF_TV_ALL", "1") != "0"
        self.fuse_adam = None
        if world_size == 1 and not opt.sdf and self.Lv == 16 and os.environ.get("N2M_FUSE_ADAM", "0") == "1":
            fl, fr = ctypes.c_uint32(0), ctypes.c_uint32(0)
            self._fuse_cap = 1 << 19
            L.call("n2m_grid_pair_fuse_plan", self._fuse_cap, self.Lv, self.ho.ctypes.data, ctypes.byref(fl), ctypes.byref(fr))
            if fl.value < self.Lv:
                self.fuse_adam = {"first_level": int(fl.value), "first_row": int(fr.value), "alt": None, "desc": {}}
                self._bwd_cfg = (2, 1.0)

    @staticmethod
    def supported(model, opt, capture=None, world_size=1):
        e1, e2 = model.encoder, model.encoder_color
        sdf = bool(opt.sdf)
        from .fused import ind_max_dim
        ind = int(getattr(opt, "ind_dim", 0))
        ind_ok = ind == 0 or (capture is not None and not sdf and world_size == 1 and ind <= ind_max_dim())
        return (bool(getattr(opt, "fused_mlp", False)) and bool(opt.fp16) and ind_ok
                and _affine(float(model.bound)) is not None and same_geometry(e1, e2) and e1.embeddings.shape[1] == 1
                and e2.embeddings.shape[1] == 2 and (sdf or not getattr(opt, "progressive_level", False))
                and opt.patch_size == 1 and (sdf or model.max_level >= e1.num_levels) and not (sdf and opt.lambda_entropy > 0)
                and not (sdf and (getattr(opt, "enable_sparse_depth", False) or getattr(opt, "enable_dense_depth", False))))

    @property
    def loss_acc(self):
        return self._loss_sum

    def _lambda_mask(self):
        if self.capture is not None and not self.capture.has_alpha:
            return 0.0
        return float(max(self.opt.lambda_mask, 0.0))

    def mark_untrained(self):
        if self.opt.mark_untrained and self.capture is not None:
            self.model.mark_untrained_grid(self.poses, self.capture.intrinsics, cam_near_far=self.cam_near_far)
        elif self.opt.mark_untrained:
            f = synthetic.LEGO_FOCAL
            self.model.mark_untrained_grid(self.poses, (f, f, synthetic.LEGO_HW / 2, synthetic.LEGO_HW / 2), cam_near_far=self.cam_near_far)

    def _ray_bufs(self, N):
        self._cur = (self._cur + 1) % len(self._bufs)
        b = self._bufs[self._cur]
        if b is None or b.cap < N:
            b = self._bufs[self._cur] = _RayBufs(max(int(N * 1.5), self._min_rays), self.device)
        return b

    def _sample_bufs(self, b, cap_m):
        if b.samples is None or b.cap_m < cap_m:
            b.cap_m = int(cap_m)
            b.samples = torch.empty(b.cap_m * 8, dtype=torch.float32, device=self.device)
        c = b.cap_m
        s = b.samples
        return s[:3 * c], s[3 * c:6 * c], s[6 * c:]

    def _work(self, M, N):
        cm, cn = self._work_cap
        if M > cm or N > cn:
            cm, cn = max(cm, int(M * 1.25) + 1024), max(cn, int(N * 1.5) + 1024, self._depth_rays)
            dev = self.device
# ... 352 lines not shown

    @torch.no_grad()
    def sync_parameters(self, density_only=False, moments=False):
        if not self.shard:
            return
        self._wait_gather()
        if self.peer is not None:
            self.peer.check()
        done = getattr(self, "_synced", (-1, False, False))
        level = (not density_only, moments)
        if done[0] == self.global_step and (done[1] or density_only) and (done[2] or not moments):
            return
        self._synced = (self.global_step, level[0] or (done[0] == self.global_step and done[1]), level[1] or (done[0] == self.global_step and done[2]))
        import torch.distributed as dist
        e1p, e2p = self.model.encoder.embeddings, self.model.encoder_color.embeddings
        tables = [(e1p.data, 1)] if density_only else [(e1p.data, 1), (e2p.data, 2)]
        if moments:
            for p, C in ((e1p, 1), (e2p, 2)):
                st = self.optimizer.state[p]
                tables += [(st["exp_avg"], C), (st["exp_avg_sq"], C)]
        for t, C in tables:
            flat = t.view(-1)
            for h, (row0, n) in self._shard_ranges().items():
                lo = 0 if h == "c" else self._split
                if h == "c" and getattr(self, "_uneven", False):
                    for r in range(self.world):
                        r0, rn = self._shard_ranges_of(r)["c"]
                        if rn > 0:
                            dist.broadcast(flat[r0 * C:(r0 + rn) * C], src=r)
                    continue
                dist.all_gather_into_tensor(flat[lo * C:(lo + self.world * n) * C], flat[row0 * C:(row0 + n) * C].clone())

    def _scaler_tail(self, participants, loss_out):
        o = self.optimizer
        gf, bf, gi = o.growth
        tail = L.ScalerTail(growth_tracker=_p(o.growth_tracker), steps=_p(o.steps), participants=participants, growth_factor=gf, backoff_factor=bf,
                            growth_interval=gi, ticket=_p(self._tail_ticket))
        if loss_out is not None:
            n_rays, buf, extra = loss_out[:3]
            ex_buf, ex_scale = extra if extra is not None else (None, 0.0)
            e2_buf, e2_n, e2_scale = loss_out[3] if len(loss_out) > 3 and loss_out[3] is not None else (None, 0, 0.0)
            tail.loss_partial, tail.n_partial, tail.n_rays, tail.loss, tail.loss_sum = _p(self._w["partial"]), (n_rays + 15) // 16, n_rays, _p(buf), _p(self._loss_sum)
            tail.extra_partial, tail.n_extra, tail.extra_scale = _p(ex_buf), self._n_spec, float(ex_scale)
            tail.extra2_partial, tail.n_extra2, tail.extra2_scale = _p(e2_buf), int(e2_n), float(e2_scale)
        return tail

    def _optimizer_step(self, full, lr_factor, loss_out=None, fused=None):
        o = self.optimizer
        self._wait_gather()
        desc, participants, groups = self._adam_desc(full, dense_only=fused is not None)
        for k, gi in enumerate(groups):
            desc.lr[k] = float(o.param_groups[gi]["initial_lr"]) * lr_factor
        b1, b2 = o.param_groups[0]["betas"]
        s = L.stream()
        peer_fused = self.peer is not None and self._peer_fused
        scaler_done = False
        if self.lookup_overlap and fused is None and not self.shard and self.Lv == 16:
            d_f, d_c = self._adam_desc_halves(full, lr_factor)
            for d in (d_f, d_c):
                L.call("n2m_adam_step", ctypes.addressof(d), float(b1), float(b2), float(o.param_groups[0]["eps"]), _p(o.scale), _p(o.found_inf),
                       _p(o.bias), s)
                if d is d_f:
                    self._fine_ready = torch.cuda.Event()
                    self._fine_ready.record()
        elif peer_fused:
            if self._adam_peer is None:
                self._adam_peer = self.peer.adam_peer([("s1", "c"), ("s2", "c"), ("s1", "f"), ("s2", "f")] + [None] * (desc.count - 4))
            L.call("n2m_adam_step_peer", ctypes.addressof(desc), float(b1), float(b2), float(o.param_groups[0]["eps"]), _p(o.scale), _p(o.found_inf),
                   _p(o.bias), ctypes.addressof(self._adam_peer), s)
        elif (self.adam_tail and loss_out is not None and fused is None and self.peer is None and not self.shard):
            tail = self._scaler_tail(participants, loss_out)
            L.call("n2m_adam_step_scaler", ctypes.addressof(desc), float(b1), float(b2), float(o.param_groups[0]["eps"]), _p(o.scale), _p(o.found_inf),
                   _p(o.bias), ctypes.addressof(tail), s)
            scaler_done = True
        else:
            L.call("n2m_adam_step", ctypes.addressof(desc), float(b1), float(b2), float(o.param_groups[0]["eps"]), _p(o.scale), _p(o.found_inf),
                   _p(o.bias), s)
        self.model.encoder_color._half_version = -1
        if fused is not None:
            L.call("n2m_adam_fuse_restore", ctypes.addressof(fused), self.ho.ctypes.data, self.Lv, _p(o.found_inf), s)
            self._fuse_swap()
        if self.peer is not None:
            for h, (row0, n) in self._shard_ranges().items():
                if peer_fused:
                    self.peer.signal_rows(h)
                else:
                    self.peer.push_rows(h, row0, n)
            self._gathers = self.peer.rows_tokens()
            if not self.chunked_gather:
                self._wait_gather()
        elif self.shard:
            self._gather_packed()
        if not scaler_done:
            tail = self._scaler_tail(participants, loss_out)
            L.call("n2m_scaler_update_slots", _p(o.scale), _p(o.found_inf), _p(o.bias), float(b1), float(b2), ctypes.addressof(tail), s)
        nxt = lr_lambda(self.global_step, self.opt.iters)
        for group in o.param_groups:
            group["lr"] = float(group["initial_lr"]) * nxt

    @torch.no_grad()
    def train_step(self):
        opt, model, dev = self.opt, self.model, self.device
        if not model.training:
            model.train()
        for g in self.optimizer.param_groups:
            g.setdefault("initial_lr", g["lr"])
        if not self._queue:
            self._fill_pipeline()
        b = self._queue.pop(0)
        self.global_step += 1
        assert b.index == self.global_step
        N = b.N
        random_bg = b.bg is not None
        bg = b.bg
        shading = SHADING["diffuse" if (self.global_step < opt.diffuse_step or opt.diffuse_only) else "full"]
        M = self._finish(b)
        self.last_num_points = M
        self.samples_seen += M
        self.rays_seen += N

        if opt.sdf:
            opt.cos_anneal_ratio = min(1, self.global_step / (0.5 * opt.iters))
            opt.normal_anneal_epsilon = 1e-1 * (1 - min(0.999, self.global_step / (0.5 * opt.iters)))
            if opt.progressive_level:
                model.max_level = 4 + int(12 * min(1, self.global_step / (0.5 * opt.iters)))
        w = self._work(max(M, 1), N)
        s = L.stream()
        c = b.cap_m
        xyzs = dirs = ts = None
        if M > 0:
            xyzs, dirs, ts = b.samples[:3 * c], b.samples[3 * c:6 * c], b.samples[6 * c:]
        o = self.optimizer
        pk = model.packed_tables()
        if self.lookup_overlap and getattr(self, "_packed", None) is not None and pk.data_ptr() != self._packed.data_ptr():
            self._fine_ready = None
        sw = self.mlp_params
        e1 = model.encoder
        seed = o.scale if self.world == 1 else o.scale / self.world
        if opt.sdf:
            return self._step_sdf(b, M, N, w, xyzs, dirs, ts, shading, seed, pk)
        fwd_terms = False
        if M > 0:
            fwd = (_p(xyzs), _p(pk), _p(e1.offsets), _p(w["h1"]), _p(w["h2"]), M, self.Lv, self.Lv, self.S, self.H0, e1.gridtype_id,
                   int(bool(e1.align_corners)), e1.interp_id, float(self.aff[0]), float(self.aff[1]))
            if self.shard and getattr(self, "_gathers", None) and self.Lv == 16:
                self._wait_gather(("c",))
                L.call("n2m_grid_encode_forward_packed_levels", *fwd, 0, 8, s)
                self._wait_gather(("f",))
                L.call("n2m_grid_encode_forward_packed_levels", *fwd, 8, 8, s)
            elif self.lookup_overlap and self._fine_ready is not None and self.Lv == 16:
                self.s_lookup.wait_event(self._fine_ready)
                with torch.cuda.stream(self.s_lookup):
                    L.call("n2m_grid_encode_forward_packed_levels", *fwd, 8, 8, L.stream())
                    done = torch.cuda.Event()
                    done.record()
                L.call("n2m_grid_encode_forward_packed_levels", *fwd, 0, 8, s)
                torch.cuda.current_stream(dev).wait_event(done)
            elif self.tv_corners and self.Lv == 16 and self.fuse_adam is None:
                L.call("n2m_grid_encode_forward_packed_tv", *fwd, _p(w["tv4"]), s)
                self._corners_of = (self.global_step, M)
            elif self.tv_fwd and self.Lv == 16 and self.fuse_adam is None:
                L.call("n2m_grid_encode_forward_packed_tvterms", *fwd, float(opt.lambda_tv), float(opt.lambda_tv * (10 if opt.bound > 1 else 1)),
                       float(0.5 / model.bound), _p(seed), _p(w["tv"]), s)
                fwd_terms = True
            else:
                self._wait_gather()
                L.call("n2m_grid_encode_forward_packed", *fwd, s)
            self._mid_step_fill()
            tv_terms = None

            def start_tv():
                go = torch.cuda.Event()
                go.record()
                self.tv_stream.wait_event(go)
                L.grid_backward_config(*self._bwd_cfg)
                with torch.cuda.stream(self.tv_stream):
                    L.call("n2m_grid_tv_terms", _p(xyzs), _p(pk) if self._bwd_cfg[0] == 2 else _p(e1.embeddings), self.ho.ctypes.data, M, self.Lv, self.S, self.H0,
                           e1.gridtype_id, int(bool(e1.align_corners)), e1.interp_id, float(opt.lambda_tv),
                           float(opt.lambda_tv * (10 if opt.bound > 1 else 1)), float(0.5 / model.bound),
                           _p(seed), float(self.aff[0]), float(self.aff[1]), _p(w["tv"]), L.stream())
                    self._tv_done = torch.cuda.Event()
                    self._tv_done.record()
            want_tv = opt.lambda_tv > 0 and self.tv_split and self.Lv == 16
            if want_tv:
                tv_terms = w["tv"]
                if self.tv_at == 0:
                    start_tv()
            elif fwd_terms:
                tv_terms = w["tv"]
                self._tv_done = None
            spec_reg = shading != 0 and opt.lambda_specular > 0
            if self.ind_dim > 0:
                codes = model.individual_codes
                L.call("n2m_field_sample_views", _p(b.rays), _p(b.views), N, M, _p(w["sview"]), s)
                L.call("n2m_field_forward_ind_train", _p(xyzs), _p(dirs) if shading != 0 else None, _p(w["h1"]), _p(w["h2"]), *[_p(p) for p in sw],
                       _p(codes), _p(w["sview"]), codes.shape[0], codes.shape[1], M, shading, 1, _p(w["sigma"]), _p(w["rgb"]), None,
                       _p(w["spec_partial"]) if spec_reg else None, s)
            else:
                L.call("n2m_field_forward_train", _p(xyzs), _p(dirs) if shading != 0 else None, _p(w["h1"]), _p(w["h2"]), *[_p(p) for p in sw], M, shading, 1,
                       _p(w["sigma"]), _p(w["rgb"]), None, _p(w["spec_partial"]) if spec_reg else None, s)
            if want_tv and self.tv_at == 1:
                start_tv()
        bg_t, bg_s = (bg, 0.0) if random_bg else (None, 1.0)
        lam_rgb, lam_mask = float(opt.lambda_rgb), self._lambda_mask()
        early = None
        d_sigma, d_rgb = w["d_sr"][:max(M, 1)], w["d_sr"][max(M, 1):4 * max(M, 1)]
        order = self.live_first and M > 0 and M <= (1 << 20) and self.peer is None
        depth_step = b.depth_view is not None or self.dense_depth is not None
        head = L.CompositeLoss(sigmas=_p(w["sigma"]), rgbs=_p(w["rgb"]), ts=_p(ts), rays=_p(b.rays), M=M, N=N, T_thresh=1e-4, gt_rgba=_p(b.rgba),
                               bg=_p(bg_t), bg_scalar=bg_s, lambda_rgb=lam_rgb, lambda_mask=lam_mask, grad_loss=_p(seed), grad_sigmas=_p(d_sigma),
                               grad_rgbs=_p(d_rgb), partial=_p(w["partial"]), lambda_entropy=float(max(opt.lambda_entropy, 0.0)),
                               live=_p(w["live"]) if order else None, block_live=_p(w["block_live"]) if order else None)
        if depth_step:
            head.gt_depth, head.depth_weight = _p(b.gtd), _p(b.dw) if b.depth_view is not None else None
            head.lambda_depth = float(opt.lambda_depth * min(1.0, self.global_step / 1000))
        L.call("n2m_composite_loss_train", ctypes.addressof(head), s)
        if order:
            L.call("n2m_sample_order_live_first", _p(b.rays), _p(w["live"]), _p(w["block_live"]), N, M, _p(w["perm"]), s)
            if self._identity_order:
                torch.arange(M, dtype=torch.int32, device=dev, out=w["perm"][:M])
        dsum = None
        if M > 0:
            if want_tv and self.tv_at == 2:
                start_tv()
            if self.marker_at == 2:
                self._marker = torch.cuda.Event(); self._marker.record()
            if self.ind_dim > 0:
                codes = model.individual_codes
                need = int(L.lib().n2m_field_ind_workspace_bytes(self._work_cap[0], codes.shape[0]))
                if self._ind_ws is None or self._ind_ws.numel() < need:
                    self._ind_ws = torch.empty(need, dtype=torch.uint8, device=dev)
                L.call("n2m_field_backward_ind_train", _p(xyzs), _p(dirs) if shading != 0 else None, _p(w["h1"]), _p(w["h2"]), *[_p(p) for p in sw],
                       _p(codes), _p(w["sview"]), codes.shape[0], codes.shape[1], M, shading, 1, _p(d_sigma), _p(d_rgb), None, _p(w["d_h1"]),
                       _p(w["d_h2"]), *[_p(g) for g in self.dw_views], _p(self.dcodes), _p(self._ind_ws), self._ind_ws.numel(), _p(o.found_inf),
                       float(2.0 * opt.lambda_specular / M) if spec_reg else 0.0, _p(seed) if spec_reg else None, s)
            else:
                if self.riders and not depth_step and self.fuse_adam is None:
                    dsum = L.DwSum()
                    L.call("n2m_field_backward_defer_dw", ctypes.addressof(dsum))
                try:
                    L.call("n2m_field_backward_train", _p(xyzs), _p(dirs) if shading != 0 else None, _p(w["h1"]), _p(w["h2"]), *[_p(p) for p in sw], M, shading, 1,
                           _p(d_sigma), _p(d_rgb), None, _p(w["d_h1"]), _p(w["d_h2"]), *[_p(g) for g in self.dw_views], _p(o.found_inf),
                           float(2.0 * opt.lambda_specular / M) if spec_reg else 0.0, _p(seed) if spec_reg else None, s)
                finally:
                    if dsum is not None:
                        L.call("n2m_field_backward_defer_dw", None)
                if dsum is not None and not dsum.partial:
                    dsum = None
            L.grid_backward_config(*self._bwd_cfg)
            need = L.lib().n2m_grid_binned_pair_workspace_bytes(M, self.Lv, self.ho.ctypes.data)
            ws = L.workspace(dev, need)
            tv = opt.lambda_tv > 0
            common = (_p(w["d_h1"]), _p(w["d_h2"]), _p(xyzs), self.ho.ctypes.data, _p(self.g1), _p(self.g2), M,
                      self.Lv, self.Lv, self.S, self.H0, e1.gridtype_id, int(bool(e1.align_corners)), e1.interp_id)
            tail = (_p(o.found_inf), float(self.aff[0]), float(self.aff[1]), 1, _p(ws), ws.numel(), s)
            fused = None
            if self.fuse_adam is not None and M <= self._fuse_cap and tv_terms is None:
                self._adam_desc(shading != 0, dense_only=True)
                fused = self._fuse_desc(lr_lambda(self.global_step - 1, opt.iters))
            if fused is not None:
                tv_args = (_p(pk) if tv else None, float(opt.lambda_tv), float(opt.lambda_tv * (10 if opt.bound > 1 else 1)),
                           float(0.5 / model.bound), _p(seed) if tv else None)
                backward = lambda half: L.call("n2m_grid_encode_backward_binned_pair_adam", *common, *tv_args, *tail[:3], _p(ws), ws.numel(),
                                               ctypes.addressof(fused), s)
            elif tv_terms is not None:
                if self._tv_done is not None:
                    torch.cuda.current_stream(dev).wait_event(self._tv_done)
                backward = lambda half: L.call("n2m_grid_encode_backward_binned_pair_tvt", *common, _p(tv_terms), *tail, half)
            else:
                tv_args = ((_p(pk) if self._bwd_cfg[0] == 2 else _p(e1.embeddings)) if tv else None, float(opt.lambda_tv),
                           float(opt.lambda_tv * (10 if opt.bound > 1 else 1)), float(0.5 / model.bound), _p(seed) if tv else None)
                backward = lambda half: (L.call("n2m_grid_encode_backward_binned_pair", *common, *tv_args, *tail) if half == 0 else
                                         L.call("n2m_grid_encode_backward_binned_pair_half", *common, *tv_args, *tail, half))
            if self.marker_at == 1:
                self._marker = torch.cuda.Event(); self._marker.record()
            if order and fused is None:
                plain_backward = backward

                def backward(half, _b=plain_backward, _perm=w["perm"]):
                    L.call("n2m_grid_backward_sample_order", _p(_perm))
                    try:
                        return _b(half)
                    finally:
                        L.call("n2m_grid_backward_sample_order", None)
            if self.peer is not None:
                self.peer.begin_step()
                L.call("n2m_grid_backward_peer_route", ctypes.byref(self._peer_route))
                try:
# ... 33 lines not shown
                carried = ctypes.c_int(0)
                if dsum is not None:
                    L.call("n2m_grid_backward_dw_rider", ctypes.addressof(dsum), ctypes.byref(carried))
                try:
                    backward(0)
                finally:
                    if use_corners:
                        L.call("n2m_grid_backward_tv_corners", None)
                    if dsum is not None:
                        L.call("n2m_grid_backward_dw_rider", None, None)
                if carried.value:
                    dsum = None
                if mid:
                    self._marker = ev
            if dsum is not None:
                L.call("n2m_field_dw_sum", ctypes.addressof(dsum), s)
        else:
            self.g1.zero_()
            self.g2.zero_()
            if self.peer is not None:
                self._wait_gather()
                self.peer.begin_step()
                self.peer.zero_slots()
                early = []
            elif self.shard:
                import torch.distributed as dist
                sp = self._split
                rs = lambda out, src: dist.reduce_scatter_tensor(out.view(-1), src.view(-1), op=dist.ReduceOp.SUM, async_op=True)
                early = [rs(self.g1s["f"], self.g1[sp:]), rs(self.g2s["f"], self.g2[sp:]), rs(self.g1s["c"], self.g1[:sp]), rs(self.g2s["c"], self.g2[:sp])]
            elif self.sync is not None and self.split_backward and self.Lv == 16:
                early = self.sync.all_reduce_sum_begin([self.g1[int(self.ho[8]):], self.g2[int(self.ho[8]):]], [])
        if self.peer is not None:
            n_dw = self.dw.numel()
            torch.cat([self.dw, o.found_inf.reshape(-1)], out=self._peer_small)
            self.peer.all_sum_small(self._peer_small)
            self.dw.copy_(self._peer_small[:n_dw])
            o.found_inf.copy_(self._peer_small[n_dw:].view_as(o.found_inf))
            for h in ("f", "c"):
                if self._peer_fused:
                    self.peer.wait_grad(h)
                else:
                    self.peer.reduce(h, self.g1s[h], self.g2s[h])
            self.peer.fold_error_into(o.found_inf)
            self.peer.raise_if_failed()
        elif self.shard:
            token = self.sync.all_reduce_sum_begin([], [self.dw, o.found_inf])
            for w_ in early:
                w_.wait()
            self.sync.all_reduce_sum_end(token)
        elif self.sync is not None:
            if early is not None:
                split = int(self.ho[8])
                token = self.sync.all_reduce_sum_begin([self.g1[:split], self.g2[:split]], [self.dw, o.found_inf])
                self.sync.all_reduce_sum_end(early)
            else:
                token = self.sync.all_reduce_sum_begin([self.g1, self.g2], [self.dw, o.found_inf])
            self.sync.all_reduce_sum_end(token)
        if self.marker_at == 0 or M == 0 or (self.marker_at == 3 and not (M > 0 and self.sync is None and fused is None and tv_terms is None)):
            self._marker = torch.cuda.Event()
            self._marker.record()
        extra = (w["spec_partial"], float(opt.lambda_specular / M)) if (M > 0 and shading != 0 and opt.lambda_specular > 0) else None
        self._lr_step(shading != 0, loss_out=(N, b.loss, extra), fused=fused if M > 0 else None)
        loss = b.loss.view(())
        self._fill_pipeline()
        return loss

    def _sdf_buf(self, M=0):
        cap = getattr(self, "_sdf_cap", 0)
        if not hasattr(self, "_sdf") or M > cap:
            cap = max(cap, int(M * 1.25) + 1024)
            dev = self.device
            f = lambda n: torch.empty(n, dtype=torch.float32, device=dev)
            old = getattr(self, "_sdf", None)
            self._sdf = {"pts": f(18 * cap), "pts01": f(18 * cap), "h6": f(16 * 6 * cap), "d_h6": f(16 * 6 * cap), "s6": f(6 * cap), "d_s6": f(6 * cap),
                         "alpha": f(cap), "d_sdf": f(cap), "x01": f(3 * cap), "eik": f((cap + 255) // 256 + 1), "varp": f((cap + 255) // 256 + 1),
                         "d_var": old["d_var"] if old is not None else torch.zeros(1, dtype=torch.float32, device=dev),
                         "fold_cnt": old["fold_cnt"] if old is not None else torch.zeros(2, 32, dtype=torch.int32, device=dev),
                         "fold_host": old["fold_host"] if old is not None else torch.zeros(32, dtype=torch.int32).pin_memory()}
            self._sdf.pop("fold", None)
            self._sdf_cap = cap
        return self._sdf

    def _step_sdf(self, b, M, N, w, xyzs, dirs, ts, shading, seed, pk):
        opt, model, dev, o = self.opt, self.model, self.device, self.optimizer
        s = L.stream()
        e1 = model.encoder
        sw = self.mlp_params
        ml = int(min(model.max_level, self.Lv))
        eps, car = float(opt.normal_anneal_epsilon), float(opt.cos_anneal_ratio)
        random_bg = b.bg is not None
        bg_t, bg_s = (b.bg, 0.0) if random_bg else (None, 1.0)
        lam_rgb, lam_mask = float(opt.lambda_rgb), self._lambda_mask()
        sb = self._sdf_buf(M)
        d_sigma, d_rgb = w["d_sr"][:max(M, 1)], w["d_sr"][max(M, 1):4 * max(M, 1)]
        extra = extra2 = None
        if M > 0:
# ... 77 lines not shown
                if K > 0:
                    L.call("n2m_sdf_fold_gather", _p(sb["d_h6"]), M, ml, _p(fb["src"]), _p(fb["pts"]), fb["cap"],
                           sb["fold_cnt"].data_ptr() + 128 * par, K, _p(fb["g"]), s)
                    L.call("n2m_grid_encode_backward_binned_lists", _p(fb["g"]), _p(fb["pts"]), fb["cap"], self.ho.ctypes.data, _p(self.g1), K, self.Lv, ml,
                           self.S, self.H0, e1.gridtype_id, int(bool(e1.align_corners)), e1.interp_id, _p(o.found_inf), 0, _p(ws), ws.numel(), s)
            else:
                L.call("n2m_grid_encode_backward_binned_pair", *batch_args, s)
                L.call("n2m_grid_encode_backward_binned_pair", _p(sb["d_h6"]), None, _p(sb["pts01"]), self.ho.ctypes.data, _p(self.g1), None, M6, *geo,
                       None, 0.0, 0.0, 1.0, None, _p(o.found_inf), 1.0, 0.0, 0, _p(ws), ws.numel(), s)
            if opt.lambda_tv > 0 and not tv_fold:
                x01 = sb["x01"][:3 * M]
                torch.add(xyzs[:3 * M], float(model.bound), out=x01)
                x01.div_(2.0 * float(model.bound))
                need_tv = L.lib().n2m_grid_binned_workspace_bytes(M, 3, 1, self.Lv, self.ho.ctypes.data, L.F32, 1)
                ws_tv = L.workspace(dev, need_tv, 1)
                L.call("n2m_grad_total_variation_binned", _p(x01), _p(e1.embeddings), _p(self.g1), self.ho.ctypes.data, tv_w, tv_wo,
                       float(0.5 / model.bound), _p(seed), M, 3, 1, self.Lv, self.S, self.H0, e1.gridtype_id, int(bool(e1.align_corners)),
                       _p(ws_tv), ws_tv.numel(), s)
            if spec_reg:
                extra = (w["spec_partial"], float(opt.lambda_specular / M))
            if lam_eik > 0:
                extra2 = (sb["eik"], (M + 255) // 256, float(lam_eik / M))
        else:
            self.g1.zero_()
            self.g2.zero_()
            sb["d_var"].zero_()
        self._marker = torch.cuda.Event()
        self._marker.record()
        self._lr_step(True if shading != 0 else False, loss_out=(N, b.loss, extra, extra2))
        loss = b.loss.view(())
        self._fill_pipeline()
        return loss

    def _lr_step(self, full, loss_out=None, fused=None):
        if full is not None:
            self._optimizer_step(full, lr_lambda(self.global_step - 1, self.opt.iters), loss_out, fused)
        if self.ema is not None and self.global_step % self.epoch_len == 0:
            self.ema_update()

    def ema_update(self):
        if self.shard:
            self.sync_parameters()
        self.ema.update()

    def averaged_parameters(self):
        import contextlib
        if self.ema is None:
            return contextlib.nullcontext()
        self.sync_parameters()
        return self.ema.average_parameters()

    @torch.no_grad()
    def eval_psnr(self, cam=0, downscale=4, use_ema=False, capture=None):
        from .trainer import Stage0Trainer
        self.sync_parameters()
        if use_ema and self.ema is not None:
            with self.averaged_parameters():
                return Stage0Trainer.eval_psnr(self, cam, downscale, capture=capture)
        return Stage0Trainer.eval_psnr(self, cam, downscale, capture=capture)
```

### nerf2mesh_amd/optim.py

```python
import ctypes

import torch

from . import _lib as L


class FusedAdamAMP(torch.optim.Optimizer):
    def __init__(self, params, lr=1e-3, betas=(0.9, 0.999), eps=1e-8, amp=True, init_scale=65536.0, growth_factor=2.0, backoff_factor=0.5,
                 growth_interval=2000):
        super().__init__(params, dict(lr=lr, betas=betas, eps=eps))
        ps = [p for g in self.param_groups for p in g["params"]]
        if len(ps) > L.ADAM_MAX:
            raise ValueError(f"FusedAdamAMP handles at most {L.ADAM_MAX} tensors per step (got {len(ps)})")
        dev = ps[0].device
        if dev.type != "cuda" or any(p.dtype != torch.float32 or not p.is_contiguous() for p in ps):
            raise ValueError("FusedAdamAMP needs contiguous fp32 CUDA parameters")
        self.amp = bool(amp)
        self.scale = torch.full((), float(init_scale) if amp else 1.0, device=dev)
        self.growth_tracker = torch.zeros((), device=dev)
        self.found_inf = torch.zeros((), device=dev)
        self.steps = torch.zeros(1 + L.ADAM_MAX, device=dev)
        self.step_count = self.steps[0]
        self.growth = (float(growth_factor), float(backoff_factor), float(growth_interval))
        b1, b2 = betas
        self.bias = torch.tensor([[1.0 - b1, (1.0 - b2) ** 0.5]] * (1 + L.ADAM_MAX), dtype=torch.float32).to(dev)
        self._slot = {p: 1 + i for i, p in enumerate(ps)}
        self._one = torch.ones((), device=dev)
        for p in ps:
            self.state[p] = dict(exp_avg=torch.zeros_like(p), exp_avg_sq=torch.zeros_like(p))
        self.shadows = {}
        self.half_grads = {}
        self.ext_grads = {}

    def state_dict(self):
        if getattr(self, "shard_sync", None) is not None:
            self.shard_sync()
        sd = super().state_dict()
        sd["n2m_amp"] = {"steps": self.steps.detach().cpu().clone(), "scale": float(self.scale), "growth_tracker": float(self.growth_tracker),
                         "amp": self.amp, "growth": self.growth}
        return sd

    def load_state_dict(self, state_dict):
        state_dict = dict(state_dict)
        extra = state_dict.pop("n2m_amp", None)
        super().load_state_dict(state_dict)
        if extra is not None:
            self.steps.copy_(extra["steps"].to(self.steps.device))
            self.scale.fill_(extra["scale"])
            self.growth_tracker.fill_(extra["growth_tracker"])
            self.growth = tuple(extra.get("growth", self.growth))
            b1, b2 = self.param_groups[0]["betas"]
            t = self.steps.double().cpu() + 1
            bias = torch.stack([1.0 - torch.tensor(b1, dtype=torch.float64) ** t, (1.0 - torch.tensor(b2, dtype=torch.float64) ** t).sqrt()], dim=1)
            self.bias.copy_(bias.float().to(self.bias.device))
        self.found_inf.zero_()
# ... 69 lines not shown
```

Measured before the change: 474.2 million samples/s.

## Defer scaler update into next field-forward launch and derive TV scale on device

The end-of-step AMP scaler/bias update kernel becomes a rider: it is deferred and run by an extra block appended to the next training field-forward launch, which removes one small serial kernel launch per step. Because the scale is then updated late, the TV-term grid forward computes the next scale on device from the tracker and found_inf, and optimizer state tensors get access hooks that flush any pending update. Double-buffered scaler slots and specular partials keep reads and writes apart. This adds a lot of bookkeeping and risks ordering bugs if a pending update is observed before it is flushed.

```diff
diff --git a/include/n2m_hip.h b/include/n2m_hip.h
--- a/include/n2m_hip.h
+++ b/include/n2m_hip.h
@@ -160,6 +160,8 @@
                                            uint32_t gridtype, int align_corners, uint32_t interp, float in_scale, float in_offset,
                                            float tv_weight, float tv_weight_outer, float tv_inner01, const float* tv_scale,
                                            float* tv_out, void* stream);
+typedef struct { const float* growth_tracker; const float* found_inf; float growth_factor, backoff_factor, growth_interval; } N2mScaleRule;
+int n2m_grid_forward_tv_scale_rule(const N2mScaleRule* rule);
 int n2m_grid_backward_tv_corners(const float* tv_corners);
 
 int n2m_grid_encode_forward_packed_levels(const float* inputs, const void* packed, const int32_t* offsets, float* outputs1,
@@ -464,6 +466,7 @@
 int n2m_ema_update(const N2mEmaDesc* desc, float one_minus_decay, void* stream);
 
 #define N2M_TAIL_TICKET_WORDS (64 * 32)
+typedef struct { float* scale; float* growth_tracker; float* found_inf; float* steps; float* bias; } N2mScalerSlot;
 typedef struct {
     float* growth_tracker; float* steps;
     uint32_t participants; float growth_factor, backoff_factor, growth_interval;
@@ -471,6 +474,7 @@
     const float* extra_partial; uint32_t n_extra; float extra_scale;
     const float* extra2_partial; uint32_t n_extra2; float extra2_scale;
     uint32_t* ticket;
+    N2mScalerSlot read, write;
 } N2mScalerTail;
 int n2m_scaler_update_slots(float* scale, float* found_inf, float* bias, double beta1, double beta2, const N2mScalerTail* tail, void* stream);
 
diff --git a/include/n2m_mlp.h b/include/n2m_mlp.h
--- a/include/n2m_mlp.h
+++ b/include/n2m_mlp.h
@@ -2,6 +2,7 @@
 #define N2M_MLP_H
 
 #include <stdint.h>
+#include "n2m_hip.h"
 
 #ifdef __cplusplus
 extern "C" {
@@ -30,6 +31,9 @@
                              float* d_w_sigma1, float* d_w_color0, float* d_w_color1, float* d_w_color2, float* d_w_spec0,
                              float* d_w_spec1, float* found_inf, float spec_reg, const float* seed, void* stream);
 uint32_t n2m_field_spec_partials(void);
+
+int n2m_field_forward_scaler_rider(const N2mScalerTail* tail, double beta1, double beta2, int* carried);
+int n2m_field_forward_scaler_pending(int* pending);
 
 typedef struct N2mDwSum {
     const float* partial;
diff --git a/nerf2mesh_amd/_lib.py b/nerf2mesh_amd/_lib.py
--- a/nerf2mesh_amd/_lib.py
+++ b/nerf2mesh_amd/_lib.py
@@ -145,6 +145,9 @@
     "n2m_field_forward_train": [_vp] * 11 + [_u32, _int, _int] + [_vp] * 5,
     "n2m_field_backward_train": [_vp] * 11 + [_u32, _int, _int] + [_vp] * 13 + [_f32, _vp, _vp],
     "n2m_field_spec_partials": [],
+    "n2m_field_forward_scaler_rider": [_vp, ctypes.c_double, ctypes.c_double, _vp],
+    "n2m_field_forward_scaler_pending": [_vp],
+    "n2m_grid_forward_tv_scale_rule": [_vp],
     "n2m_field_backward_defer_dw": [_vp],
     "n2m_field_dw_sum": [_vp, _vp],
     "n2m_grid_backward_dw_rider": [_vp, _vp],
@@ -208,11 +211,19 @@
                 ("shadow_mode", _i32 * ADAM_MAX), ("clear_grad", _i32 * ADAM_MAX), ("slot", _i32 * ADAM_MAX), ("count", _u32)]
 
 
+class ScalerSlot(ctypes.Structure):
+    _fields_ = [("scale", _vp), ("growth_tracker", _vp), ("found_inf", _vp), ("steps", _vp), ("bias", _vp)]
+
+
+class ScaleRule(ctypes.Structure):
+    _fields_ = [("growth_tracker", _vp), ("found_inf", _vp), ("growth_factor", _f32), ("backoff_factor", _f32), ("growth_interval", _f32)]
+
+
 class ScalerTail(ctypes.Structure):
     _fields_ = [("growth_tracker", _vp), ("steps", _vp), ("participants", _u32), ("growth_factor", _f32), ("backoff_factor", _f32),
                 ("growth_interval", _f32), ("loss_partial", _vp), ("n_partial", _u32), ("n_rays", _u32), ("loss", _vp), ("loss_sum", _vp),
                 ("extra_partial", _vp), ("n_extra", _u32), ("extra_scale", _f32), ("extra2_partial", _vp), ("n_extra2", _u32),
-                ("extra2_scale", _f32), ("ticket", _vp)]
+                ("extra2_scale", _f32), ("ticket", _vp), ("read", ScalerSlot), ("write", ScalerSlot)]
 
 
 class DwSum(ctypes.Structure):
diff --git a/nerf2mesh_amd/csrc/gridencoder.hip b/nerf2mesh_amd/csrc/gridencoder.hip
--- a/nerf2mesh_amd/csrc/gridencoder.hip
+++ b/nerf2mesh_amd/csrc/gridencoder.hip
@@ -8,6 +8,7 @@
 #include "../../include/n2m_peer.h"
 #include "../../include/n2m_mlp.h"
 #include "n2m_dw_sum.hpp"
+#include "n2m_scaler.hpp"
 
 namespace {
 
@@ -400,6 +401,15 @@
     if (tv.table && tv.scale_ptr) { const float s = *tv.scale_ptr; wi *= s; wo *= s; }
     w_in = wi / 6.0f; w_out = wo / 6.0f;
 }
+struct TvScaleRule { const float* tracker; const float* found_inf; float growth_factor, backoff_factor, growth_interval; };
+__device__ __forceinline__ void tv_weights_derived(const TvParams& tv, const TvScaleRule& r, float& w_in, float& w_out) {
+    if (!(r.found_inf && tv.table && tv.scale_ptr)) { tv_weights(tv, w_in, w_out); return; }
+    float wi = tv.weight, wo = tv.weight_outer, tracker_next;
+    const float s = n2m_scale_next(*tv.scale_ptr, r.tracker ? *r.tracker : 0.0f, *r.found_inf == 0.0f, r.tracker != nullptr, r.growth_factor,
+                                   r.backoff_factor, r.growth_interval, tracker_next);
+    wi *= s; wo *= s;
+    w_in = wi / 6.0f; w_out = wo / 6.0f;
+}
 __device__ __forceinline__ bool tv_inner(const TvParams& tv, const float (&x)[3]) {
     return fmaxf(fmaxf(fabsf(x[0] - 0.5f), fabsf(x[1] - 0.5f)), fabsf(x[2] - 0.5f)) <= tv.inner01;
 }
@@ -419,7 +429,7 @@
                             float* __restrict__ out1, _Float16* __restrict__ out2, uint32_t B, uint32_t max_level, LevelTable lv,
                             uint32_t gridtype, bool align_corners, uint32_t interp, uint32_t n_tiles, float in_scale, float in_offset,
                             uint32_t xcd_group, uint32_t level_begin, uint32_t n_levels, float4* __restrict__ tv4, TvParams tv,
-                            float* __restrict__ tv_out) {
+                            float* __restrict__ tv_out, TvScaleRule tv_rule) {
     __builtin_amdgcn_s_setprio(3);
     constexpr uint32_t D = 3;
     typedef _Float16 h2 __attribute__((ext_vector_type(2)));
@@ -526,7 +536,7 @@
     }
     if constexpr (TVT) {
         float w_in, w_out;
-        tv_weights(tv, w_in, w_out);
+        tv_weights_derived(tv, tv_rule, w_in, w_out);
         const float w = tv_inner(tv, x) ? w_in : w_out;
         float tvv;
         if (tv_fast) {
@@ -4256,7 +4266,7 @@
 static int forward_packed(const float* inputs, const void* packed, const int32_t* offsets, float* outputs1, void* outputs2, uint32_t B, uint32_t L,
                           uint32_t max_level, float S, uint32_t H, uint32_t gridtype, int align_corners, uint32_t interp, float in_scale, float in_offset,
                           void* stream, uint32_t level_begin, uint32_t n_levels, float* tv_corners = nullptr, const TvParams* tvp = nullptr,
-                          float* tv_out = nullptr);
+                          float* tv_out = nullptr, const TvScaleRule* rule = nullptr);
 
 extern "C" int n2m_grid_encode_forward_packed(const float* inputs, const void* packed, const int32_t* offsets, float* outputs1, void* outputs2,
                                               uint32_t B, uint32_t L, uint32_t max_level, float S, uint32_t H, uint32_t gridtype,
@@ -4277,7 +4287,8 @@
 
 static int forward_packed(const float* inputs, const void* packed, const int32_t* offsets, float* outputs1, void* outputs2, uint32_t B, uint32_t L,
                           uint32_t max_level, float S, uint32_t H, uint32_t gridtype, int align_corners, uint32_t interp, float in_scale, float in_offset,
-                          void* stream, uint32_t level_begin, uint32_t n_levels, float* tv_corners, const TvParams* tvp, float* tv_out) {
+                          void* stream, uint32_t level_begin, uint32_t n_levels, float* tv_corners, const TvParams* tvp, float* tv_out,
+                          const TvScaleRule* rule) {
     const char* fn = "grid_encode_forward_packed";
     if (int rc = check_dims(fn, 3, 2, L, max_level, N2M_F16)) return rc;
     N2M_REQUIRE(inputs && packed && offsets && outputs1, N2M_ENULL, "%s: NULL tensor", fn);
@@ -4298,11 +4309,11 @@
         tv.stride = 2u;
         N2M_LAUNCH(grid_forward3_packed_kernel<true>, blocks, 256, 0, s, inputs, (const uint2*)packed, offsets, outputs1, (_Float16*)outputs2, B,
                    level_begin + n_levels, lv, gridtype, align_corners != 0, interp, n_tiles, in_scale, in_offset, xg, level_begin, n_levels,
-                   (float4*)nullptr, tv, tv_out);
+                   (float4*)nullptr, tv, tv_out, rule ? *rule : TvScaleRule{});
     } else {
         N2M_LAUNCH(grid_forward3_packed_kernel<false>, blocks, 256, 0, s, inputs, (const uint2*)packed, offsets, outputs1, (_Float16*)outputs2, B,
                    level_begin + n_levels, lv, gridtype, align_corners != 0, interp, n_tiles, in_scale, in_offset, xg, level_begin, n_levels,
-                   reinterpret_cast<float4*>(tv_corners), TvParams{}, (float*)nullptr);
+                   reinterpret_cast<float4*>(tv_corners), TvParams{}, (float*)nullptr, TvScaleRule{});
     }
     N2M_CHECK_LAUNCH();
     return 0;
@@ -4316,15 +4327,26 @@
                           0u, max_level < L ? max_level : L, tv_corners);
 }
 
+static thread_local TvScaleRule g_tv_scale_rule{};
+extern "C" int n2m_grid_forward_tv_scale_rule(const N2mScaleRule* r) {
+    if (r == nullptr) { g_tv_scale_rule = TvScaleRule{}; return 0; }
+    N2M_REQUIRE(r->found_inf != nullptr, N2M_ENULL, "n2m_grid_forward_tv_scale_rule: NULL found_inf");
+    g_tv_scale_rule = TvScaleRule{r->growth_tracker, r->found_inf, r->growth_factor, r->backoff_factor, r->growth_interval};
+    return 0;
+}
+
 extern "C" int n2m_grid_encode_forward_packed_tvterms(const float* inputs, const void* packed, const int32_t* offsets, float* outputs1, void* outputs2,
                                                       uint32_t B, uint32_t L, uint32_t max_level, float S, uint32_t H, uint32_t gridtype,
                                                       int align_corners, uint32_t interp, float in_scale, float in_offset, float tv_weight,
                                                       float tv_weight_outer, float tv_inner01, const float* tv_scale, float* tv_out, void* stream) {
+    const TvScaleRule rule = g_tv_scale_rule;
+    g_tv_scale_rule = TvScaleRule{};
     N2M_REQUIRE(tv_out != nullptr, N2M_ENULL, "grid_encode_forward_packed_tvterms: NULL tv_out");
     N2M_REQUIRE(max_level == L, N2M_EINVAL, "grid_encode_forward_packed_tvterms: TV terms need max_level == L (every level of tv_out is written)");
+    N2M_REQUIRE(rule.found_inf == nullptr || tv_scale != nullptr, N2M_ENULL, "grid_encode_forward_packed_tvterms: a scale rule without the scale it starts from");
     const TvParams tv{nullptr, tv_weight, tv_weight_outer, tv_inner01, tv_scale, 2u};
     return forward_packed(inputs, packed, offsets, outputs1, outputs2, B, L, max_level, S, H, gridtype, align_corners, interp, in_scale, in_offset, stream,
-                          0u, L, nullptr, &tv, tv_out);
+                          0u, L, nullptr, &tv, tv_out, rule.found_inf ? &rule : nullptr);
 }
 
 extern "C" int n2m_debug_fill_times(int on, unsigned long long* out) {
diff --git a/nerf2mesh_amd/csrc/mlp.hip b/nerf2mesh_amd/csrc/mlp.hip
--- a/nerf2mesh_amd/csrc/mlp.hip
+++ b/nerf2mesh_amd/csrc/mlp.hip
@@ -4,6 +4,7 @@
 #include "n2m_common.hpp"
 #include "../../include/n2m_mlp.h"
 #include "n2m_dw_sum.hpp"
+#include "n2m_scaler.hpp"
 
 namespace {
 
@@ -382,14 +383,14 @@
 }
 
 template <bool DO_DENSITY, bool DO_COLOR, bool IND = false>
-__global__ void __launch_bounds__(256) field_forward_kernel(typename ArgsOf<IND>::type a) {
+__device__ __forceinline__ void field_forward_body(const typename ArgsOf<IND>::type& a, const uint32_t n_blocks) {
     __builtin_amdgcn_s_setprio(3);
     extern __shared__ __attribute__((aligned(16))) _Float16 lds[];
     stage_images<256, false, DO_DENSITY, DO_COLOR, IND>(lds, a);
     if constexpr (IND) stage_color0_ind<false>(lds + O_C0X_FWD, nullptr, a.w[2], a.ind.D);
 
     const int lane = threadIdx.x & 63, n = lane & 31, g = lane >> 5;
-    const uint32_t wave = blockIdx.x * 4 + (threadIdx.x >> 6), n_waves = gridDim.x * 4;
+    const uint32_t wave = blockIdx.x * 4 + (threadIdx.x >> 6), n_waves = n_blocks * 4;
     const uint32_t n_tiles = (a.M + 31) / 32;
     RawTile nxt;
     float spec_sq = 0.f;
@@ -470,8 +471,20 @@
         __syncthreads();
         if (threadIdx.x == 0) a.spec_sq_partial[blockIdx.x] = ((spec_wave[0] + spec_wave[1]) + spec_wave[2]) + spec_wave[3];
         if (blockIdx.x == 0)
-            for (int i = (int)gridDim.x + (int)threadIdx.x; i < kSpecPartials; i += 256) a.spec_sq_partial[i] = 0.f;
-    }
+            for (int i = (int)n_blocks + (int)threadIdx.x; i < kSpecPartials; i += 256) a.spec_sq_partial[i] = 0.f;
+    }
+}
+template <bool DO_DENSITY, bool DO_COLOR, bool IND = false>
+__global__ void __launch_bounds__(256) field_forward_kernel(typename ArgsOf<IND>::type a) {
+    field_forward_body<DO_DENSITY, DO_COLOR, IND>(a, gridDim.x);
+}
+template <bool DO_DENSITY, bool DO_COLOR>
+__global__ void __launch_bounds__(256) field_forward_scaler_kernel(FieldArgs a, ScalerTailK k) {
+    if (blockIdx.x == gridDim.x - 1u) {
+        scaler_update_slots_body<false>(k);
+        return;
+    }
+    field_forward_body<DO_DENSITY, DO_COLOR, false>(a, gridDim.x - 1u);
 }
 
 __device__ __forceinline__ void tile_put(_Float16* tile, int kb, const h4& f, int lane) {
@@ -1171,10 +1184,26 @@
 
 }
 
+struct ScalerRider { bool armed; ScalerTailK k; int* carried; };
+static thread_local ScalerRider g_scaler_rider{};
+extern "C" int n2m_field_forward_scaler_rider(const N2mScalerTail* tail, double beta1, double beta2, int* carried) {
+    if (tail == nullptr) { g_scaler_rider = ScalerRider{}; return 0; }
+    N2M_REQUIRE(carried != nullptr, N2M_ENULL, "n2m_field_forward_scaler_rider: NULL carried");
+    N2M_REQUIRE(!g_scaler_rider.armed, N2M_EINVAL, "n2m_field_forward_scaler_rider: an update handed over earlier was never launched (disarm it, or launch it)");
+    if (int rc = scaler_check_tail("n2m_field_forward_scaler_rider", nullptr, nullptr, nullptr, tail, true)) return rc;
+    g_scaler_rider = ScalerRider{true, scaler_tail_k(nullptr, nullptr, nullptr, beta1, beta2, tail), carried};
+    return 0;
+}
+extern "C" int n2m_field_forward_scaler_pending(int* pending) {
+    N2M_REQUIRE(pending != nullptr, N2M_ENULL, "n2m_field_forward_scaler_pending: NULL pending");
+    *pending = g_scaler_rider.armed ? 1 : 0;
+    return 0;
+}
+
 static int field_forward_impl(const float* xyz, const float* dirs, const float* h1, const void* h2, const float* w_sigma0,
                                  const float* w_sigma1, const float* w_color0, const float* w_color1, const float* w_color2,
                                  const float* w_spec0, const float* w_spec1, uint32_t M, int shading, int normalize_dirs, float* sigma, float* rgb,
-                                 float* specular, float* spec_sq_partial, void* stream, const IndArgs* ind = nullptr) {
+                                 float* specular, float* spec_sq_partial, void* stream, const IndArgs* ind = nullptr, bool train = false) {
     const float* w[7] = {w_sigma0, w_sigma1, w_color0, w_color1, w_color2, w_spec0, w_spec1};
     const bool density = sigma != nullptr;
     if (int rc = check_field("field_forward", xyz, h1, w, density, shading)) return rc;
@@ -1203,6 +1232,16 @@
         N2M_CHECK_LAUNCH();
         return 0;
     }
+    if (train && color && density && g_scaler_rider.armed) {
+        const ScalerRider r = g_scaler_rider;
+        g_scaler_rider = ScalerRider{};
+        N2M_REQUIRE(r.k.extra_partial == nullptr || r.k.extra_partial != a.spec_sq_partial, N2M_EINVAL,
+                    "field_forward: the scaler rider reads the specular partials this launch writes (alternate two arrays)");
+        N2M_LAUNCH((field_forward_scaler_kernel<true, true>), persistent_grid(M) * 2 + 1, 256, smem, s, a, r.k);
+        N2M_CHECK_LAUNCH();
+        *r.carried = 1;
+        return 0;
+    }
     if (color && density) N2M_LAUNCH((field_forward_kernel<true, true>), persistent_grid(M) * 2, 256, smem, s, a);
     else if (color) N2M_LAUNCH((field_forward_kernel<false, true>), persistent_grid(M) * 2, 256, smem, s, a);
     else N2M_LAUNCH((field_forward_kernel<true, false>), persistent_grid(M) * 2, 256, smem, s, a);
@@ -1222,7 +1261,7 @@
                                        const float* w_spec0, const float* w_spec1, uint32_t M, int shading, int normalize_dirs, float* sigma,
                                        float* rgb, float* specular, float* spec_sq_partial, void* stream) {
     return field_forward_impl(xyz, dirs, h1, h2, w_sigma0, w_sigma1, w_color0, w_color1, w_color2, w_spec0, w_spec1, M, shading, normalize_dirs,
-                              sigma, rgb, specular, spec_sq_partial, stream);
+                              sigma, rgb, specular, spec_sq_partial, stream, nullptr, true);
 }
 extern "C" uint32_t n2m_field_spec_partials(void) { return (uint32_t)kSpecPartials; }
 
diff --git a/nerf2mesh_amd/csrc/n2m_scaler.hpp b/nerf2mesh_amd/csrc/n2m_scaler.hpp
--- /dev/null
+++ b/nerf2mesh_amd/csrc/n2m_scaler.hpp
@@ -0,0 +1,162 @@
+#pragma once
+#include <hip/hip_runtime.h>
+#include <stdint.h>
+#include "../../include/n2m_hip.h"
+#include "n2m_common.hpp"
+
+__device__ __forceinline__ float n2m_scale_next(float scale, float tracker, bool ok, bool tracked, float growth_factor, float backoff_factor,
+                                                float growth_interval, float& tracker_next) {
+    tracker_next = tracker;
+    if (!ok) {
+        tracker_next = 0.0f;
+        return scale * backoff_factor;
+    }
+    if (tracked) {
+        const float g = tracker + 1.0f;
+        if (g >= growth_interval) {
+            const float ns = scale * growth_factor;
+            tracker_next = 0.0f;
+            return ns <= 3.0e38f ? ns : scale;
+        }
+        tracker_next = g;
+    }
+    return scale;
+}
+
+struct ScalerSlotK { float* scale; float* growth_tracker; float* found_inf; float* steps; float* bias; };
+struct ScalerTailK {
+    ScalerSlotK r, w;
+    uint32_t participants; double beta1, beta2; float growth_factor, backoff_factor, growth_interval;
+    const float* loss_partial; uint32_t n_partial; float inv_rays; float* loss; float* loss_sum;
+    const float* extra_partial; uint32_t n_extra; float extra_scale;
+    const float* extra2_partial; uint32_t n_extra2; float extra2_scale;
+    uint32_t* ticket;
+};
+
+template <bool ONE_WAVE>
+__device__ __forceinline__ void scaler_update_slots_body(const ScalerTailK& k) {
+    const uint32_t s = ONE_WAVE ? (threadIdx.x & 63u) : threadIdx.x;
+    float tot_part = 0.0f, tot_extra = 0.0f, tot_extra2 = 0.0f;
+    bool ok;
+    if constexpr (ONE_WAVE) {
+        auto sum256 = [&](const float* __restrict__ part, uint32_t n) {
+            float acc[4] = {0.0f, 0.0f, 0.0f, 0.0f};
+            for (uint32_t base = 0; base < n; base += 2048u) {
+                float x[8][4];
+#pragma unroll
+                for (uint32_t k = 0; k < 8u; ++k)
+#pragma unroll
+                    for (uint32_t w = 0; w < 4u; ++w) {
+                        const uint32_t i = base + 256u * k + 64u * w + s;
+                        x[k][w] = i < n ? part[i] : 0.0f;
+                    }
+#pragma unroll
+                for (uint32_t k = 0; k < 8u; ++k)
+#pragma unroll
+                    for (uint32_t w = 0; w < 4u; ++w)
+                        if (base + 256u * k + 64u * w + s < n) acc[w] += x[k][w];
+            }
+            float tot = 0.0f;
+#pragma unroll
+            for (uint32_t w = 0; w < 4u; ++w) tot += n2m_wave_sum(acc[w]);
+            return tot;
+        };
+        if (k.extra2_partial) tot_extra2 = sum256(k.extra2_partial, k.n_extra2);
+        if (k.extra_partial) tot_extra = sum256(k.extra_partial, k.n_extra);
+        if (k.loss_partial) tot_part = sum256(k.loss_partial, k.n_partial);
+        ok = *k.r.found_inf == 0.0f;
+    } else {
+        __shared__ float wave_part[16], wave_extra[16], wave_extra2[16];
+        if (k.extra2_partial) {
+            float acc = 0.0f;
+            for (uint32_t i = s; i < k.n_extra2; i += blockDim.x) acc += k.extra2_partial[i];
+            acc = n2m_wave_sum(acc);
+            if ((s & 63u) == 0u) wave_extra2[s >> 6] = acc;
+        }
+        if (k.extra_partial) {
+            float acc = 0.0f;
+            for (uint32_t i = s; i < k.n_extra; i += blockDim.x) acc += k.extra_partial[i];
+            acc = n2m_wave_sum(acc);
+            if ((s & 63u) == 0u) wave_extra[s >> 6] = acc;
+        }
+        if (k.loss_partial) {
+            float acc = 0.0f;
+            for (uint32_t i = s; i < k.n_partial; i += blockDim.x) acc += k.loss_partial[i];
+            acc = n2m_wave_sum(acc);
+            if ((s & 63u) == 0u) wave_part[s >> 6] = acc;
+        }
+        ok = *k.r.found_inf == 0.0f;
+        __syncthreads();
+        if (s == 0) {
+            for (uint32_t w = 0; w < (blockDim.x + 63u) / 64u; ++w) {
+                if (k.loss_partial) tot_part += wave_part[w];
+                if (k.extra_partial) tot_extra += wave_extra[w];
+                if (k.extra2_partial) tot_extra2 += wave_extra2[w];
+            }
+        }
+    }
+    if (k.loss_partial && s == 0) {
+        float v = tot_part * k.inv_rays;
+        if (k.extra_partial) v += tot_extra * k.extra_scale;
+        if (k.extra2_partial) v += tot_extra2 * k.extra2_scale;
+        if (k.loss) *k.loss = v;
+        if (k.loss_sum) *k.loss_sum += v;
+    }
+    if (s == 0) {
+        if (k.r.scale) {
+            float tracker_next = 0.0f;
+            const float tracker = k.r.growth_tracker ? *k.r.growth_tracker : 0.0f;
+            *k.w.scale = n2m_scale_next(*k.r.scale, tracker, ok, k.r.growth_tracker != nullptr, k.growth_factor, k.backoff_factor, k.growth_interval,
+                                        tracker_next);
+            if (k.r.growth_tracker) *k.w.growth_tracker = tracker_next;
+        }
+        *k.w.found_inf = 0.0f;
+    }
+    if (s <= N2M_ADAM_MAX) {
+        float n = k.r.steps[s];
+        if (ok && (s == 0 || ((k.participants >> (s - 1u)) & 1u))) n += 1.0f;
+        k.w.steps[s] = n;
+        const double t = (double)n + 1.0;
+        k.w.bias[2u * s] = (float)(1.0 - pow(k.beta1, t));
+        k.w.bias[2u * s + 1u] = (float)sqrt(1.0 - pow(k.beta2, t));
+    }
+}
+
+static ScalerTailK scaler_tail_k(float* scale, float* found_inf, float* bias, double beta1, double beta2, const N2mScalerTail* t) {
+    const bool lp = t->loss_partial != nullptr;
+    const float* e1 = lp ? t->extra_partial : nullptr;
+    const float* e2 = lp ? t->extra2_partial : nullptr;
+    const ScalerSlotK here{scale, t->growth_tracker, found_inf, t->steps, bias};
+    const bool two = t->read.found_inf != nullptr;
+    const ScalerSlotK r = two ? ScalerSlotK{t->read.scale, t->read.growth_tracker, t->read.found_inf, t->read.steps, t->read.bias} : here;
+    const ScalerSlotK w = two ? ScalerSlotK{t->write.scale, t->write.growth_tracker, t->write.found_inf, t->write.steps, t->write.bias} : here;
+    return ScalerTailK{r, w, t->participants, beta1, beta2, t->growth_factor, t->backoff_factor,
+                       t->growth_interval, t->loss_partial, lp ? t->n_partial : 0u, lp ? 1.0f / (float)t->n_rays : 0.0f, lp ? t->loss : nullptr,
+                       lp ? t->loss_sum : nullptr, e1, e1 ? t->n_extra : 0u, t->extra_scale, e2, e2 ? t->n_extra2 : 0u, t->extra2_scale, t->ticket};
+}
+
+static int scaler_check_tail(const char* fn, const float* scale, const float* found_inf, const float* bias, const N2mScalerTail* t, bool two_slots) {
+    N2M_REQUIRE(t != nullptr, N2M_ENULL, "%s: NULL tail", fn);
+    const bool named = t->read.found_inf != nullptr || t->write.found_inf != nullptr;
+    N2M_REQUIRE(named || !two_slots, N2M_ENULL, "%s: NULL slot pointers (tail.read / tail.write)", fn);
+    if (named) {
+        const N2mScalerSlot* sl[2] = {&t->read, &t->write};
+        for (int i = 0; i < 2; ++i) {
+            N2M_REQUIRE(sl[i]->found_inf != nullptr && sl[i]->steps != nullptr && sl[i]->bias != nullptr, N2M_ENULL,
+                        "%s: NULL found_inf / steps / bias in the %s slot", fn, i ? "write" : "read");
+            N2M_REQUIRE(sl[i]->scale != nullptr || sl[i]->growth_tracker == nullptr, N2M_ENULL, "%s: a growth tracker needs a scale", fn);
+        }
+        N2M_REQUIRE((t->read.scale != nullptr) == (t->write.scale != nullptr) && (t->read.growth_tracker != nullptr) == (t->write.growth_tracker != nullptr),
+                    N2M_EINVAL, "%s: scale / growth tracker in one slot only", fn);
+        const bool same = t->read.found_inf == t->write.found_inf;
+        N2M_REQUIRE(same == (t->read.steps == t->write.steps) && same == (t->read.bias == t->write.bias) && same == (t->read.scale == t->write.scale || !t->read.scale) &&
+                    same == (t->read.growth_tracker == t->write.growth_tracker || !t->read.growth_tracker), N2M_EINVAL,
+                    "%s: the read and the write slot share some arrays and not others", fn);
+        N2M_REQUIRE(!(two_slots && same), N2M_EINVAL, "%s: the rider needs a write slot other than the read slot (it runs beside kernels that read the read slot)", fn);
+    } else {
+        N2M_REQUIRE(found_inf != nullptr && t->steps != nullptr && bias != nullptr, N2M_ENULL, "%s: NULL found_inf / steps / bias", fn);
+        N2M_REQUIRE(scale != nullptr || t->growth_tracker == nullptr, N2M_ENULL, "%s: a growth tracker needs a scale", fn);
+    }
+    N2M_REQUIRE(t->loss_partial == nullptr || t->n_rays > 0, N2M_EINVAL, "%s: the loss partials need the ray count", fn);
+    return 0;
+}
diff --git a/nerf2mesh_amd/csrc/step_helpers.hip b/nerf2mesh_amd/csrc/step_helpers.hip
--- a/nerf2mesh_amd/csrc/step_helpers.hip
+++ b/nerf2mesh_amd/csrc/step_helpers.hip
@@ -2,6 +2,7 @@
 
 #include "n2m_common.hpp"
 #include "../../include/n2m_peer.h"
+#include "n2m_scaler.hpp"
 
 namespace {
 
@@ -869,107 +870,6 @@
     adam_body<PEER>(t, beta1, beta2, omb1, omb2, eps, scale, found_inf, bias, pe);
 }
 
-struct ScalerTailK {
-    float* scale; float* growth_tracker; float* found_inf; float* steps; float* bias;
-    uint32_t participants; double beta1, beta2; float growth_factor, backoff_factor, growth_interval;
-    const float* loss_partial; uint32_t n_partial; float inv_rays; float* loss; float* loss_sum;
-    const float* extra_partial; uint32_t n_extra; float extra_scale;
-    const float* extra2_partial; uint32_t n_extra2; float extra2_scale;
-    uint32_t* ticket;
-};
-
-template <bool ONE_WAVE>
-__device__ __forceinline__ void scaler_update_slots_body(const ScalerTailK& k) {
-    const uint32_t s = ONE_WAVE ? (threadIdx.x & 63u) : threadIdx.x;
-    float tot_part = 0.0f, tot_extra = 0.0f, tot_extra2 = 0.0f;
-    bool ok;
-    if constexpr (ONE_WAVE) {
-        auto sum256 = [&](const float* __restrict__ part, uint32_t n) {
-            float acc[4] = {0.0f, 0.0f, 0.0f, 0.0f};
-            for (uint32_t base = 0; base < n; base += 2048u) {
-                float x[8][4];
-#pragma unroll
-                for (uint32_t k = 0; k < 8u; ++k)
-#pragma unroll
-                    for (uint32_t w = 0; w < 4u; ++w) {
-                        const uint32_t i = base + 256u * k + 64u * w + s;
-                        x[k][w] = i < n ? part[i] : 0.0f;
-                    }
-#pragma unroll
-                for (uint32_t k = 0; k < 8u; ++k)
-#pragma unroll
-                    for (uint32_t w = 0; w < 4u; ++w)
-                        if (base + 256u * k + 64u * w + s < n) acc[w] += x[k][w];
-            }
-            float tot = 0.0f;
-#pragma unroll
-            for (uint32_t w = 0; w < 4u; ++w) tot += n2m_wave_sum(acc[w]);
-            return tot;
-        };
-        if (k.extra2_partial) tot_extra2 = sum256(k.extra2_partial, k.n_extra2);
-        if (k.extra_partial) tot_extra = sum256(k.extra_partial, k.n_extra);
-        if (k.loss_partial) tot_part = sum256(k.loss_partial, k.n_partial);
-        ok = *k.found_inf == 0.0f;
-    } else {
-        __shared__ float wave_part[16], wave_extra[16], wave_extra2[16];
-        if (k.extra2_partial) {
-            float acc = 0.0f;
-            for (uint32_t i = s; i < k.n_extra2; i += blockDim.x) acc += k.extra2_partial[i];
-            acc = n2m_wave_sum(acc);
-            if ((s & 63u) == 0u) wave_extra2[s >> 6] = acc;
-        }
-        if (k.extra_partial) {
-            float acc = 0.0f;
-            for (uint32_t i = s; i < k.n_extra; i += blockDim.x) acc += k.extra_partial[i];
-            acc = n2m_wave_sum(acc);
-            if ((s & 63u) == 0u) wave_extra[s >> 6] = acc;
-        }
-        if (k.loss_partial) {
-            float acc = 0.0f;
-            for (uint32_t i = s; i < k.n_partial; i += blockDim.x) acc += k.loss_partial[i];
-            acc = n2m_wave_sum(acc);
-            if ((s & 63u) == 0u) wave_part[s >> 6] = acc;
-        }
-        ok = *k.found_inf == 0.0f;
-        __syncthreads();
-        if (s == 0) {
-            for (uint32_t w = 0; w < (blockDim.x + 63u) / 64u; ++w) {
-                if (k.loss_partial) tot_part += wave_part[w];
-                if (k.extra_partial) tot_extra += wave_extra[w];
-                if (k.extra2_partial) tot_extra2 += wave_extra2[w];
-            }
-        }
-    }
-    if (k.loss_partial && s == 0) {
-        float v = tot_part * k.inv_rays;
-        if (k.extra_partial) v += tot_extra * k.extra_scale;
-        if (k.extra2_partial) v += tot_extra2 * k.extra2_scale;
-        if (k.loss) *k.loss = v;
-        if (k.loss_sum) *k.loss_sum += v;
-    }
-    if (s == 0) {
-        if (!ok) {
-            if (k.scale) *k.scale *= k.backoff_factor;
-            if (k.growth_tracker) *k.growth_tracker = 0.0f;
-        } else if (k.growth_tracker) {
-            const float g = *k.growth_tracker + 1.0f;
-            if (g >= k.growth_interval) {
-                const float ns = *k.scale * k.growth_factor;
-                if (k.scale && ns <= 3.0e38f) *k.scale = ns;
-                *k.growth_tracker = 0.0f;
-            } else {
-                *k.growth_tracker = g;
-            }
-        }
-        *k.found_inf = 0.0f;
-    }
-    if (s <= N2M_ADAM_MAX) {
-        if (ok && (s == 0 || ((k.participants >> (s - 1u)) & 1u))) k.steps[s] += 1.0f;
-        const double t = (double)k.steps[s] + 1.0;
-        k.bias[2u * s] = (float)(1.0 - pow(k.beta1, t));
-        k.bias[2u * s + 1u] = (float)sqrt(1.0 - pow(k.beta2, t));
-    }
-}
 
 
 constexpr uint32_t kTailSlots = 64;
@@ -1006,14 +906,6 @@
     scaler_update_slots_body<true>(k);
 }
 
-static ScalerTailK scaler_tail_k(float* scale, float* found_inf, float* bias, double beta1, double beta2, const N2mScalerTail* t) {
-    const bool lp = t->loss_partial != nullptr;
-    const float* e1 = lp ? t->extra_partial : nullptr;
-    const float* e2 = lp ? t->extra2_partial : nullptr;
-    return ScalerTailK{scale, t->growth_tracker, found_inf, t->steps, bias, t->participants, beta1, beta2, t->growth_factor, t->backoff_factor,
-                       t->growth_interval, t->loss_partial, lp ? t->n_partial : 0u, lp ? 1.0f / (float)t->n_rays : 0.0f, lp ? t->loss : nullptr,
-                       lp ? t->loss_sum : nullptr, e1, e1 ? t->n_extra : 0u, t->extra_scale, e2, e2 ? t->n_extra2 : 0u, t->extra2_scale, t->ticket};
-}
 
 static int adam_step_impl(const N2mAdamDesc* d, double beta1, double beta2, float eps, const float* scale, const float* found_inf,
                           const float* bias, const N2mAdamPeer* peer, void* stream, const N2mScalerTail* tail = nullptr) {
@@ -1142,9 +1034,7 @@
 
 extern "C" int n2m_scaler_update_slots(float* scale, float* found_inf, float* bias, double beta1, double beta2, const N2mScalerTail* tail,
                                        void* stream) {
-    N2M_REQUIRE(tail != nullptr, N2M_ENULL, "scaler_update_slots: NULL tail");
-    N2M_REQUIRE(found_inf != nullptr && tail->steps != nullptr && bias != nullptr, N2M_ENULL, "scaler_update_slots: NULL found_inf / steps / bias");
-    N2M_REQUIRE(tail->loss_partial == nullptr || tail->n_rays > 0, N2M_EINVAL, "scaler_update_slots: the loss partials need the ray count");
+    if (int rc = scaler_check_tail("scaler_update_slots", scale, found_inf, bias, tail, false)) return rc;
     scaler_update_slots_kernel<<<1, tail->loss_partial ? 256 : 64, 0, (hipStream_t)stream>>>(scaler_tail_k(scale, found_inf, bias, beta1, beta2, tail));
     N2M_CHECK_LAUNCH();
     return 0;
diff --git a/nerf2mesh_amd/engine.py b/nerf2mesh_amd/engine.py
--- a/nerf2mesh_amd/engine.py
+++ b/nerf2mesh_amd/engine.py
@@ -1,6 +1,7 @@
 import ctypes
 import os
 import time
+import types
 
 import numpy as np
 import torch
@@ -57,6 +58,25 @@
         self.N = 0
         self.args = None
         self.refreshed = False
+
+
+class _PendingLoss(torch.Tensor):
+
+    @staticmethod
+    def of(t, flush):
+        out = t.as_subclass(_PendingLoss)
+        out._n2m_flush = flush
+        return out
+
+    @classmethod
+    def __torch_function__(cls, func, types, args=(), kwargs=None):
+        for a in args:
+            flush = getattr(a, "__dict__", {}).get("_n2m_flush") if isinstance(a, _PendingLoss) else None
+            if flush is not None:
+                flush()
+        with torch._C.DisableTorchFunctionSubclass():
+            out = func(*args, **(kwargs or {}))
+        return out.as_subclass(torch.Tensor) if isinstance(out, _PendingLoss) else out
 
 
 class Stage0Engine:
@@ -217,6 +237,17 @@
             if fl.value < self.Lv:
                 self.fuse_adam = {"first_level": int(fl.value), "first_row": int(fr.value), "alt": None, "desc": {}}
                 self._bwd_cfg = (2, 1.0)
+        self.scaler_rider = (self.riders and self.tv_fwd and self.fuse_adam is None and not self.adam_tail and not self.lookup_overlap
+                             and self.Lv == 16 and self.sync is None and self.peer is None and not self.shard)
+        self._pending = None
+        self._sslot = 0
+        self._slots = [self.optimizer.raw_state()] if hasattr(self.optimizer, "raw_state") else None
+        if self._slots is None:
+            self.scaler_rider = False
+        if self.scaler_rider:
+            self._slots.append({k: torch.zeros_like(v) for k, v in self._slots[0].items()})
+            self._spec_alt = [torch.zeros(self._n_spec, dtype=torch.float32, device=dev) for _ in range(2)]
+            self.optimizer._before_state_access = self._flush_scaler
 
     @staticmethod
     def supported(model, opt, capture=None, world_size=1):
@@ -233,7 +264,32 @@
 
     @property
     def loss_acc(self):
+        self._flush_scaler()
         return self._loss_sum
+
+    def _st(self):
+        return self._slots[self._sslot] if self._slots is not None else {k: getattr(self.optimizer, k) for k in ("scale", "growth_tracker", "found_inf", "steps", "bias")}
+
+    @staticmethod
+    def _slot_of(st):
+        return L.ScalerSlot(scale=_p(st["scale"]), growth_tracker=_p(st["growth_tracker"]), found_inf=_p(st["found_inf"]), steps=_p(st["steps"]),
+                            bias=_p(st["bias"]))
+
+    def _update_scaler(self, tail, betas, read):
+        st = self._slots[read] if self._slots is not None else self._st()
+        if read != 0:
+            tail.read, tail.write = self._slot_of(st), self._slot_of(self._slots[0])
+        else:
+            tail.read, tail.write = L.ScalerSlot(), L.ScalerSlot()
+        L.call("n2m_scaler_update_slots", _p(st["scale"]), _p(st["found_inf"]), _p(st["bias"]), float(betas[0]), float(betas[1]), ctypes.addressof(tail),
+               L.stream())
+        self._sslot = 0
+
+    def _flush_scaler(self):
+        pend = self._pending
+        if pend is not None:
+            self._pending = None
+            self._update_scaler(pend["tail"], pend["betas"], pend["read"])
 
     def _lambda_mask(self):
         if self.capture is not None and not self.capture.has_alpha:
@@ -652,9 +708,9 @@
                 dist.all_gather_into_tensor(flat[lo * C:(lo + self.world * n) * C], flat[row0 * C:(row0 + n) * C].clone())
 
     def _scaler_tail(self, participants, loss_out):
-        o = self.optimizer
+        o, st = self.optimizer, self._st()
         gf, bf, gi = o.growth
-        tail = L.ScalerTail(growth_tracker=_p(o.growth_tracker), steps=_p(o.steps), participants=participants, growth_factor=gf, backoff_factor=bf,
+        tail = L.ScalerTail(growth_tracker=_p(st["growth_tracker"]), steps=_p(st["steps"]), participants=participants, growth_factor=gf, backoff_factor=bf,
                             growth_interval=gi, ticket=_p(self._tail_ticket))
         if loss_out is not None:
             n_rays, buf, extra = loss_out[:3]
@@ -663,10 +719,13 @@
             tail.loss_partial, tail.n_partial, tail.n_rays, tail.loss, tail.loss_sum = _p(self._w["partial"]), (n_rays + 15) // 16, n_rays, _p(buf), _p(self._loss_sum)
             tail.extra_partial, tail.n_extra, tail.extra_scale = _p(ex_buf), self._n_spec, float(ex_scale)
             tail.extra2_partial, tail.n_extra2, tail.extra2_scale = _p(e2_buf), int(e2_n), float(e2_scale)
+            tail._keep = (self._w["partial"], buf, ex_buf, e2_buf)
         return tail
 
-    def _optimizer_step(self, full, lr_factor, loss_out=None, fused=None):
+    def _optimizer_step(self, full, lr_factor, loss_out=None, fused=None, defer=False):
         o = self.optimizer
+        st = self._st()
+        o_ = types.SimpleNamespace(scale=st["scale"], found_inf=st["found_inf"], bias=st["bias"])
         self._wait_gather()
         desc, participants, groups = self._adam_desc(full, dense_only=fused is not None)
         for k, gi in enumerate(groups):
@@ -678,27 +737,27 @@
         if self.lookup_overlap and fused is None and not self.shard and self.Lv == 16:
             d_f, d_c = self._adam_desc_halves(full, lr_factor)
             for d in (d_f, d_c):
-                L.call("n2m_adam_step", ctypes.addressof(d), float(b1), float(b2), float(o.param_groups[0]["eps"]), _p(o.scale), _p(o.found_inf),
-                       _p(o.bias), s)
+                L.call("n2m_adam_step", ctypes.addressof(d), float(b1), float(b2), float(o.param_groups[0]["eps"]), _p(o_.scale), _p(o_.found_inf),
+                       _p(o_.bias), s)
                 if d is d_f:
                     self._fine_ready = torch.cuda.Event()
                     self._fine_ready.record()
         elif peer_fused:
             if self._adam_peer is None:
                 self._adam_peer = self.peer.adam_peer([("s1", "c"), ("s2", "c"), ("s1", "f"), ("s2", "f")] + [None] * (desc.count - 4))
-            L.call("n2m_adam_step_peer", ctypes.addressof(desc), float(b1), float(b2), float(o.param_groups[0]["eps"]), _p(o.scale), _p(o.found_inf),
-                   _p(o.bias), ctypes.addressof(self._adam_peer), s)
+            L.call("n2m_adam_step_peer", ctypes.addressof(desc), float(b1), float(b2), float(o.param_groups[0]["eps"]), _p(o_.scale), _p(o_.found_inf),
+                   _p(o_.bias), ctypes.addressof(self._adam_peer), s)
         elif (self.adam_tail and loss_out is not None and fused is None and self.peer is None and not self.shard):
             tail = self._scaler_tail(participants, loss_out)
-            L.call("n2m_adam_step_scaler", ctypes.addressof(desc), float(b1), float(b2), float(o.param_groups[0]["eps"]), _p(o.scale), _p(o.found_inf),
-                   _p(o.bias), ctypes.addressof(tail), s)
+            L.call("n2m_adam_step_scaler", ctypes.addressof(desc), float(b1), float(b2), float(o.param_groups[0]["eps"]), _p(o_.scale), _p(o_.found_inf),
+                   _p(o_.bias), ctypes.addressof(tail), s)
             scaler_done = True
         else:
-            L.call("n2m_adam_step", ctypes.addressof(desc), float(b1), float(b2), float(o.param_groups[0]["eps"]), _p(o.scale), _p(o.found_inf),
-                   _p(o.bias), s)
+            L.call("n2m_adam_step", ctypes.addressof(desc), float(b1), float(b2), float(o.param_groups[0]["eps"]), _p(o_.scale), _p(o_.found_inf),
+                   _p(o_.bias), s)
         self.model.encoder_color._half_version = -1
         if fused is not None:
-            L.call("n2m_adam_fuse_restore", ctypes.addressof(fused), self.ho.ctypes.data, self.Lv, _p(o.found_inf), s)
+            L.call("n2m_adam_fuse_restore", ctypes.addressof(fused), self.ho.ctypes.data, self.Lv, _p(o_.found_inf), s)
             self._fuse_swap()
         if self.peer is not None:
             for h, (row0, n) in self._shard_ranges().items():
@@ -713,7 +772,10 @@
             self._gather_packed()
         if not scaler_done:
             tail = self._scaler_tail(participants, loss_out)
-            L.call("n2m_scaler_update_slots", _p(o.scale), _p(o.found_inf), _p(o.bias), float(b1), float(b2), ctypes.addressof(tail), s)
+            if defer:
+                self._pending = {"tail": tail, "betas": (b1, b2), "read": self._sslot}
+            else:
+                self._update_scaler(tail, (b1, b2), self._sslot)
         nxt = lr_lambda(self.global_step, self.opt.iters)
         for group in o.param_groups:
             group["lr"] = float(group["initial_lr"]) * nxt
@@ -751,12 +813,21 @@
         if M > 0:
             xyzs, dirs, ts = b.samples[:3 * c], b.samples[3 * c:6 * c], b.samples[6 * c:]
         o = self.optimizer
+        depth_step = b.depth_view is not None or self.dense_depth is not None
+        can_ride = self.scaler_rider and M > 0 and not depth_step and self.ind_dim == 0 and not opt.sdf
+        if self._pending is not None and not can_ride:
+            self._flush_scaler()
+        pend = self._pending
+        st_read = self._slots[pend["read"]] if pend is not None else None
+        if pend is not None:
+            self._sslot = 1 - pend["read"]
+        st = self._st()
         pk = model.packed_tables()
         if self.lookup_overlap and getattr(self, "_packed", None) is not None and pk.data_ptr() != self._packed.data_ptr():
             self._fine_ready = None
         sw = self.mlp_params
         e1 = model.encoder
-        seed = o.scale if self.world == 1 else o.scale / self.world
+        seed = st["scale"] if self.world == 1 else st["scale"] / self.world
         if opt.sdf:
             return self._step_sdf(b, M, N, w, xyzs, dirs, ts, shading, seed, pk)
         fwd_terms = False
@@ -780,8 +851,15 @@
                 L.call("n2m_grid_encode_forward_packed_tv", *fwd, _p(w["tv4"]), s)
                 self._corners_of = (self.global_step, M)
             elif self.tv_fwd and self.Lv == 16 and self.fuse_adam is None:
-                L.call("n2m_grid_encode_forward_packed_tvterms", *fwd, float(opt.lambda_tv), float(opt.lambda_tv * (10 if opt.bound > 1 else 1)),
-                       float(0.5 / model.bound), _p(seed), _p(w["tv"]), s)
+                if pend is not None:
+                    rule = L.ScaleRule(_p(st_read["growth_tracker"]), _p(st_read["found_inf"]), *o.growth)
+                    L.call("n2m_grid_forward_tv_scale_rule", ctypes.addressof(rule))
+                try:
+                    L.call("n2m_grid_encode_forward_packed_tvterms", *fwd, float(opt.lambda_tv), float(opt.lambda_tv * (10 if opt.bound > 1 else 1)),
+                           float(0.5 / model.bound), _p(seed if pend is None else st_read["scale"]), _p(w["tv"]), s)
+                finally:
+                    if pend is not None:
+                        L.call("n2m_grid_forward_tv_scale_rule", None)
                 fwd_terms = True
             else:
                 self._wait_gather()
@@ -810,15 +888,29 @@
                 tv_terms = w["tv"]
                 self._tv_done = None
             spec_reg = shading != 0 and opt.lambda_specular > 0
+            spec_buf = self._spec_alt[self.global_step & 1] if self.scaler_rider else w["spec_partial"]
             if self.ind_dim > 0:
                 codes = model.individual_codes
                 L.call("n2m_field_sample_views", _p(b.rays), _p(b.views), N, M, _p(w["sview"]), s)
                 L.call("n2m_field_forward_ind_train", _p(xyzs), _p(dirs) if shading != 0 else None, _p(w["h1"]), _p(w["h2"]), *[_p(p) for p in sw],
                        _p(codes), _p(w["sview"]), codes.shape[0], codes.shape[1], M, shading, 1, _p(w["sigma"]), _p(w["rgb"]), None,
-                       _p(w["spec_partial"]) if spec_reg else None, s)
+                       _p(spec_buf) if spec_reg else None, s)
             else:
-                L.call("n2m_field_forward_train", _p(xyzs), _p(dirs) if shading != 0 else None, _p(w["h1"]), _p(w["h2"]), *[_p(p) for p in sw], M, shading, 1,
-                       _p(w["sigma"]), _p(w["rgb"]), None, _p(w["spec_partial"]) if spec_reg else None, s)
+                rode = ctypes.c_int(0)
+                if pend is not None:
+                    tail = pend["tail"]
+                    tail.read, tail.write = self._slot_of(st_read), self._slot_of(st)
+                    L.call("n2m_field_forward_scaler_rider", ctypes.addressof(tail), float(pend["betas"][0]), float(pend["betas"][1]), ctypes.byref(rode))
+                try:
+                    L.call("n2m_field_forward_train", _p(xyzs), _p(dirs) if shading != 0 else None, _p(w["h1"]), _p(w["h2"]), *[_p(p) for p in sw], M, shading, 1,
+                           _p(w["sigma"]), _p(w["rgb"]), None, _p(spec_buf) if spec_reg else None, s)
+                finally:
+                    if pend is not None:
+                        L.call("n2m_field_forward_scaler_rider", None, 0.0, 0.0, None)
+                if pend is not None:
+                    if not rode.value:
+                        L.call("n2m_scaler_update_slots", None, None, None, float(pend["betas"][0]), float(pend["betas"][1]), ctypes.addressof(tail), s)
+                    self._pending = pend = None
             if want_tv and self.tv_at == 1:
                 start_tv()
         bg_t, bg_s = (bg, 0.0) if random_bg else (None, 1.0)
@@ -826,7 +918,6 @@
         early = None
         d_sigma, d_rgb = w["d_sr"][:max(M, 1)], w["d_sr"][max(M, 1):4 * max(M, 1)]
         order = self.live_first and M > 0 and M <= (1 << 20) and self.peer is None
-        depth_step = b.depth_view is not None or self.dense_depth is not None
         head = L.CompositeLoss(sigmas=_p(w["sigma"]), rgbs=_p(w["rgb"]), ts=_p(ts), rays=_p(b.rays), M=M, N=N, T_thresh=1e-4, gt_rgba=_p(b.rgba),
                                bg=_p(bg_t), bg_scalar=bg_s, lambda_rgb=lam_rgb, lambda_mask=lam_mask, grad_loss=_p(seed), grad_sigmas=_p(d_sigma),
                                grad_rgbs=_p(d_rgb), partial=_p(w["partial"]), lambda_entropy=float(max(opt.lambda_entropy, 0.0)),
@@ -852,7 +943,7 @@
                     self._ind_ws = torch.empty(need, dtype=torch.uint8, device=dev)
                 L.call("n2m_field_backward_ind_train", _p(xyzs), _p(dirs) if shading != 0 else None, _p(w["h1"]), _p(w["h2"]), *[_p(p) for p in sw],
                        _p(codes), _p(w["sview"]), codes.shape[0], codes.shape[1], M, shading, 1, _p(d_sigma), _p(d_rgb), None, _p(w["d_h1"]),
-                       _p(w["d_h2"]), *[_p(g) for g in self.dw_views], _p(self.dcodes), _p(self._ind_ws), self._ind_ws.numel(), _p(o.found_inf),
+                       _p(w["d_h2"]), *[_p(g) for g in self.dw_views], _p(self.dcodes), _p(self._ind_ws), self._ind_ws.numel(), _p(st["found_inf"]),
                        float(2.0 * opt.lambda_specular / M) if spec_reg else 0.0, _p(seed) if spec_reg else None, s)
             else:
                 if self.riders and not depth_step and self.fuse_adam is None:
@@ -860,7 +951,7 @@
                     L.call("n2m_field_backward_defer_dw", ctypes.addressof(dsum))
                 try:
                     L.call("n2m_field_backward_train", _p(xyzs), _p(dirs) if shading != 0 else None, _p(w["h1"]), _p(w["h2"]), *[_p(p) for p in sw], M, shading, 1,
-                           _p(d_sigma), _p(d_rgb), None, _p(w["d_h1"]), _p(w["d_h2"]), *[_p(g) for g in self.dw_views], _p(o.found_inf),
+                           _p(d_sigma), _p(d_rgb), None, _p(w["d_h1"]), _p(w["d_h2"]), *[_p(g) for g in self.dw_views], _p(st["found_inf"]),
                            float(2.0 * opt.lambda_specular / M) if spec_reg else 0.0, _p(seed) if spec_reg else None, s)
                 finally:
                     if dsum is not None:
@@ -873,7 +964,7 @@
             tv = opt.lambda_tv > 0
             common = (_p(w["d_h1"]), _p(w["d_h2"]), _p(xyzs), self.ho.ctypes.data, _p(self.g1), _p(self.g2), M,
                       self.Lv, self.Lv, self.S, self.H0, e1.gridtype_id, int(bool(e1.align_corners)), e1.interp_id)
-            tail = (_p(o.found_inf), float(self.aff[0]), float(self.aff[1]), 1, _p(ws), ws.numel(), s)
+            tail = (_p(st["found_inf"]), float(self.aff[0]), float(self.aff[1]), 1, _p(ws), ws.numel(), s)
             fused = None
             if self.fuse_adam is not None and M <= self._fuse_cap and tv_terms is None:
                 self._adam_desc(shading != 0, dense_only=True)
@@ -973,36 +1064,39 @@
                 early = self.sync.all_reduce_sum_begin([self.g1[int(self.ho[8]):], self.g2[int(self.ho[8]):]], [])
         if self.peer is not None:
             n_dw = self.dw.numel()
-            torch.cat([self.dw, o.found_inf.reshape(-1)], out=self._peer_small)
+            torch.cat([self.dw, st["found_inf"].reshape(-1)], out=self._peer_small)
             self.peer.all_sum_small(self._peer_small)
             self.dw.copy_(self._peer_small[:n_dw])
-            o.found_inf.copy_(self._peer_small[n_dw:].view_as(o.found_inf))
+            st["found_inf"].copy_(self._peer_small[n_dw:].view_as(st["found_inf"]))
             for h in ("f", "c"):
                 if self._peer_fused:
                     self.peer.wait_grad(h)
                 else:
                     self.peer.reduce(h, self.g1s[h], self.g2s[h])
-            self.peer.fold_error_into(o.found_inf)
+            self.peer.fold_error_into(st["found_inf"])
             self.peer.raise_if_failed()
         elif self.shard:
-            token = self.sync.all_reduce_sum_begin([], [self.dw, o.found_inf])
+            token = self.sync.all_reduce_sum_begin([], [self.dw, st["found_inf"]])
             for w_ in early:
                 w_.wait()
             self.sync.all_reduce_sum_end(token)
         elif self.sync is not None:
             if early is not None:
                 split = int(self.ho[8])
-                token = self.sync.all_reduce_sum_begin([self.g1[:split], self.g2[:split]], [self.dw, o.found_inf])
+                token = self.sync.all_reduce_sum_begin([self.g1[:split], self.g2[:split]], [self.dw, st["found_inf"]])
                 self.sync.all_reduce_sum_end(early)
             else:
-                token = self.sync.all_reduce_sum_begin([self.g1, self.g2], [self.dw, o.found_inf])
+                token = self.sync.all_reduce_sum_begin([self.g1, self.g2], [self.dw, st["found_inf"]])
             self.sync.all_reduce_sum_end(token)
         if self.marker_at == 0 or M == 0 or (self.marker_at == 3 and not (M > 0 and self.sync is None and fused is None and tv_terms is None)):
             self._marker = torch.cuda.Event()
             self._marker.record()
-        extra = (w["spec_partial"], float(opt.lambda_specular / M)) if (M > 0 and shading != 0 and opt.lambda_specular > 0) else None
-        self._lr_step(shading != 0, loss_out=(N, b.loss, extra), fused=fused if M > 0 else None)
+        extra = (spec_buf, float(opt.lambda_specular / M)) if (M > 0 and shading != 0 and opt.lambda_specular > 0) else None
+        self._lr_step(shading != 0, loss_out=(N, b.loss, extra), fused=fused if M > 0 else None, defer=can_ride)
         loss = b.loss.view(())
+        if self._pending is not None:
+            mine = self._pending
+            loss = _PendingLoss.of(loss, lambda: self._flush_scaler() if self._pending is mine else None)
         self._fill_pipeline()
         return loss
 
@@ -1146,9 +1240,9 @@
         self._fill_pipeline()
         return loss
 
-    def _lr_step(self, full, loss_out=None, fused=None):
+    def _lr_step(self, full, loss_out=None, fused=None, defer=False):
         if full is not None:
-            self._optimizer_step(full, lr_lambda(self.global_step - 1, self.opt.iters), loss_out, fused)
+            self._optimizer_step(full, lr_lambda(self.global_step - 1, self.opt.iters), loss_out, fused, defer)
         if self.ema is not None and self.global_step % self.epoch_len == 0:
             self.ema_update()
 
diff --git a/nerf2mesh_amd/optim.py b/nerf2mesh_amd/optim.py
--- a/nerf2mesh_amd/optim.py
+++ b/nerf2mesh_amd/optim.py
@@ -5,7 +5,29 @@
 from . import _lib as L
 
 
+def _state_tensor(name):
+    key = "_n2m_" + name
+
+    def get(self):
+        if self._before_state_access is not None:
+            self._before_state_access()
+        return self.__dict__[key]
+
+    def put(self, value):
+        if self._before_state_access is not None:
+            self._before_state_access()
+        self.__dict__[key] = value
+    return property(get, put)
+
+
 class FusedAdamAMP(torch.optim.Optimizer):
+    _before_state_access = None
+    scale, growth_tracker, found_inf, steps, bias = (_state_tensor(n) for n in ("scale", "growth_tracker", "found_inf", "steps", "bias"))
+    step_count = property(lambda self: self.steps[0])
+
+    def raw_state(self):
+        return {n: self.__dict__["_n2m_" + n] for n in ("scale", "growth_tracker", "found_inf", "steps", "bias")}
+
     def __init__(self, params, lr=1e-3, betas=(0.9, 0.999), eps=1e-8, amp=True, init_scale=65536.0, growth_factor=2.0, backoff_factor=0.5,
                  growth_interval=2000):
         super().__init__(params, dict(lr=lr, betas=betas, eps=eps))
@@ -20,7 +42,6 @@
         self.growth_tracker = torch.zeros((), device=dev)
         self.found_inf = torch.zeros((), device=dev)
         self.steps = torch.zeros(1 + L.ADAM_MAX, device=dev)
-        self.step_count = self.steps[0]
         self.growth = (float(growth_factor), float(backoff_factor), float(growth_interval))
         b1, b2 = betas
         self.bias = torch.tensor([[1.0 - b1, (1.0 - b2) ** 0.5]] * (1 + L.ADAM_MAX), dtype=torch.float32).to(dev)
```

Result: no change. 477.2 million samples/s (median of 6 runs) (+0.6%).
